# ZenHKD/ocr-vi-invoice

Measured on AMD Instinct MI355X. Metric: invoice images/sec end-to-end (det+rec), higher is better.
Workload: dtype f16x2

## Files before the change

### include/ocrvi.h

```cpp
#ifndef OCRVI_H
#define OCRVI_H

#include <stddef.h>
#include <stdint.h>

#ifdef __cplusplus
extern "C" {
#endif

#define OCRVI_OK 0
#define OCRVI_EINVAL (-1)
#define OCRVI_EHIP (-2)
#define OCRVI_ENOMEM (-3)
#define OCRVI_EBLOB (-4)
#define OCRVI_ERANGE (-5)

typedef enum { OCRVI_F32 = 0, OCRVI_BF16 = 1, OCRVI_F16 = 2, OCRVI_F16X2 = 3 } ocrvi_dtype;

const char* ocrvi_last_error(void);
int ocrvi_abi_version(void);

typedef struct ocrvi_det ocrvi_det;

typedef struct {
    int32_t dtype;
    float k;
    int32_t max_batch;
    int32_t backbone;
    int32_t no_dcn;
    int32_t reserved[3];
} ocrvi_det_cfg;

int ocrvi_det_create(int device, const void* blob, size_t blob_bytes, const ocrvi_det_cfg* cfg, ocrvi_det** out);
void ocrvi_det_destroy(ocrvi_det* h);
int ocrvi_det_workspace_bytes(const ocrvi_det* h, int N, int H, int W, size_t* bytes);
int ocrvi_det_forward(ocrvi_det* h, const float* x, int N, int H, int W,
                      float* binary, float* thresh, float* thresh_binary, float* bin_logits, float* thresh_logits,
                      void* workspace, size_t workspace_bytes, void* stream);
int ocrvi_det_binary_workspace_bytes(const ocrvi_det* h, int N, int H, int W, size_t* bytes);
int ocrvi_det_forward_binary(ocrvi_det* h, const float* x, int N, int H, int W, float* binary,
                             void* workspace, size_t workspace_bytes, void* stream);
int ocrvi_det_status(const ocrvi_det* h);
int ocrvi_det_debug_features(ocrvi_det* h, int N, int H, int W, float* c2, float* c3, float* c4, float* c5,
                             float* fused, void* workspace, size_t workspace_bytes, void* stream);

typedef struct ocrvi_rec ocrvi_rec;

typedef struct {
    int32_t dtype;
    int32_t dims[3];
    int32_t num_blocks[3];
    int32_t num_local[3];
    int32_t num_classes;
    int32_t blank_id;
    int32_t reserved[4];
} ocrvi_rec_cfg;

int ocrvi_rec_create(int device, const void* blob, size_t blob_bytes, const ocrvi_rec_cfg* cfg, ocrvi_rec** out);
void ocrvi_rec_destroy(ocrvi_rec* h);
int ocrvi_rec_workspace_bytes(const ocrvi_rec* h, int B, int H, int W, size_t* bytes);
int ocrvi_rec_forward(ocrvi_rec* h, const float* x, int B, int H, int W,
                      float* log_probs, int32_t* argmax_ids, int32_t* ids, int32_t* lens,
                      void* workspace, size_t workspace_bytes, void* stream);
int ocrvi_rec_status(const ocrvi_rec* h);
int ocrvi_rec_debug_features(ocrvi_rec* h, int B, int H, int W, float* backbone_norm, float* frm,
                             void* workspace, size_t workspace_bytes, void* stream);

int ocrvi_range_reset(int device, void* stream);
int ocrvi_range_flag(int device, int* raised);

int ocrvi_ctc_greedy(int device, const float* log_probs, int T, int B, int C, int blank_id,
                     int32_t* argmax_ids, int32_t* ids, int32_t* lens, void* stream);

int ocrvi_normalize_u8(int device, const uint8_t* images, int N, int H, int W, float* out, void* stream);
int ocrvi_resize_u8(int device, const uint8_t* src, int src_h, int src_w, uint8_t* dst, int dst_h, int dst_w, void* stream);
int ocrvi_crop_resize_normalize(int device, const uint8_t* images, int n_img, int H, int W, const int32_t* boxes, int B,
                                int out_h, int out_w, float* out, void* stream);

#define OCRVI_PAGE_ENTRY 4
int ocrvi_resize_normalize_pages(int device, const int64_t* pages, int n, int H, int W, float* out, void* stream);
int ocrvi_crop_resize_normalize_pages(int device, const int64_t* pages, int n_pages, const int32_t* boxes, int B, int out_h, int out_w,
                                      float* out, void* stream);

int ocrvi_four_point_transform(const double* pts , double* m_fwd , double* m_inv , int32_t* out_w, int32_t* out_h);
int ocrvi_warp_perspective_u8(int device, const uint8_t* src, int src_h, int src_w, const double* m_inv_host ,
                              uint8_t* dst, int dst_h, int dst_w, void* stream);
int ocrvi_warp_perspective_pages(int device, const int64_t* src_pages, const int64_t* dst_pages, const double* m_inv , int n,
                                 void* stream);

int ocrvi_min_area_quads(const int32_t* points, const int32_t* offs, int n, double* quads , int32_t* flags );
int ocrvi_quad_crops(const double* quads, const int32_t* flags, int n, const int32_t* page_ids, const int32_t* page_hw ,
                     int32_t* crops , double* m_inv );
int ocrvi_crop_quad_resize_normalize_pages(int device, const int64_t* pages, int n_pages, const int32_t* crops, const double* m_inv, int B,
                                           int out_h, int out_w, float* out, void* stream);
int ocrvi_crop_quad_resize_normalize(int device, const uint8_t* images, int n_img, int H, int W, const int32_t* crops, const double* m_inv,
                                     int B, int out_h, int out_w, float* out, void* stream);

int ocrvi_enhance_init(int device);
int ocrvi_enhance_tables(void* out, size_t cap, size_t* bytes);
int ocrvi_enhance_workspace_bytes(int h, int w, size_t* bytes);
int ocrvi_enhance_u8(int device, const uint8_t* src, int h, int w, uint8_t* dst, void* workspace, size_t workspace_bytes, void* stream);
int ocrvi_rgb_to_lab_u8(int device, const uint8_t* src, int h, int w, uint8_t* dst, void* stream);
int ocrvi_lab_to_rgb_u8(int device, const uint8_t* src, int h, int w, uint8_t* dst, void* stream);
#define OCRVI_CLAHE_WORKSPACE_BYTES 16384
int ocrvi_clahe_lab_u8(int device, const uint8_t* src, int h, int w, uint8_t* dst, void* workspace, size_t workspace_bytes, void* stream);
int ocrvi_nlm_lab_u8(int device, const uint8_t* src, int h, int w, uint8_t* dst, void* stream);
int ocrvi_sharpen_u8(int device, const uint8_t* src, int h, int w, uint8_t* dst, void* stream);

typedef struct {
    int32_t width, height, components;
    int32_t h_samp[3], v_samp[3];
    int32_t restart_interval;
    int32_t orientation;
    int32_t out_height, out_width;
    int32_t reserved;
    int64_t blocks;
    uint64_t stream_bytes;
    uint64_t workspace_bytes;
    uint16_t quant[3][64];
    char reason[160];
} ocrvi_jpeg_info_t;
int ocrvi_jpeg_info(const void* data, size_t n, ocrvi_jpeg_info_t* info);
int ocrvi_jpeg_parse(const void* data, size_t n, void* out, size_t cap, size_t* used);
#define OCRVI_JPEG_ENTRY 64
int ocrvi_jpeg_table_entry(const ocrvi_jpeg_info_t* info, size_t used, int64_t stream_offset, int64_t dst_offset, int64_t dst_stride,
                           int64_t workspace_offset, int64_t* entry);
int ocrvi_jpeg_decode_pages(int device, const void* records_dev, const int64_t* table_dev, int n_pages, void* dst_base, void* workspace,
                            size_t workspace_bytes, void* stream);

int ocrvi_jpeg_quant_tables(int quality, uint16_t* luma, uint16_t* chroma);
#define OCRVI_JPEG_HEADER_MAX 640
int ocrvi_jpeg_encode_header(int width, int height, int components, int subsampling, int quality, void* out, size_t cap, size_t* used);
int ocrvi_jpeg_encode_sizes(int width, int height, int components, int subsampling, int64_t* blocks, uint64_t* workspace_bytes,
                            uint64_t* scan_capacity, uint64_t* offsets);
#define OCRVI_JPEG_ENC_ENTRY 64
int ocrvi_jpeg_encode_table_entry(int width, int height, int components, int subsampling, int quality, int64_t src_offset, int64_t src_stride,
                                  int64_t out_offset, int64_t out_capacity, int64_t workspace_offset, int64_t* entry);
int ocrvi_jpeg_encode_pages(int device, const void* src_base, const int64_t* table_dev, int n_pages, void* out_base, int64_t* lengths_dev,
                            void* workspace, size_t workspace_bytes, void* stream);

#define OCRVI_OVERLAY_SEG 8
#define OCRVI_OVERLAY_PRIM 8
#define OCRVI_OVERLAY_MAX_COORD 16384
int ocrvi_overlay_segments(const int32_t* points, const int32_t* offs, const int32_t* page_boxes, const int32_t* page_pairs,
                           const int32_t* page_hw , int n_pages, uint32_t box_rgb, uint32_t label_rgb, int thickness,
                           int32_t* segs , int64_t seg_cap, int32_t* prims ,
                           int64_t prim_cap, int32_t* prim_offs , int64_t* n_segs, int64_t* n_prims);
int ocrvi_overlay_pages(int device, const int64_t* pages, int n_pages, const int32_t* prims, const int32_t* segs, const int32_t* prim_offs,
                        int max_h, int max_w, void* stream);

int ocrvi_db_postprocess(const float* prob, int H, int W, float thresh, float box_thresh, int max_candidates, float unclip_ratio,
                         float min_area, int32_t* points, int cap_points, int32_t* box_offsets, float* scores, int cap_boxes, int* n_boxes);

int ocrvi_unclip_polygon(const int32_t* pts, int n_pts, double distance, int32_t* out, int cap_pts, int* n_out);

int ocrvi_db_boxes_batch(const float* prob, int n_pages, int H, int W, float thresh, float box_thresh, int max_candidates,
                         float unclip_ratio, float min_area, double scale_w, double scale_h, int orig_h, int orig_w, int page_base,
                         int32_t* rects, float* scores, int cap_per_page, int32_t* counts, int threads);

int ocrvi_db_boxes_pages(const float* prob, int n_pages, int H, int W, float thresh, float box_thresh, int max_candidates, float unclip_ratio,
                         float min_area, const double* scale_w, const double* scale_h, const int32_t* orig_h, const int32_t* orig_w,
                         const int32_t* page_ids, int32_t* points, int cap_points, int32_t* box_offsets, int32_t* rects, float* scores,
                         int cap_per_page, int32_t* counts, int32_t* overflow, int threads);

size_t ocrvi_db_components_workspace_bytes(int n_pages, int H, int W);
int ocrvi_db_components(int device, const float* prob, int n_pages, int H, int W, float thresh, uint32_t* mask_bits, int32_t* comps,
                        int32_t* counts, int cap, long long* offsets, float* packed, long long pack_cap, void* workspace, void* stream);
int ocrvi_db_boxes_batch_sparse(const uint32_t* mask_bits, const int32_t* comps, const int32_t* comp_counts, int cap, const long long* offsets,
                                const float* packed, long long pack_cap, int n_pages, int H, int W, float box_thresh, int max_candidates,
                                float unclip_ratio, float min_area, double scale_w, double scale_h, int orig_h, int orig_w, int page_base,
                                int32_t* rects, float* scores, int cap_per_page, int32_t* counts, int threads, int32_t* skipped);

#define OCRVI_DB_TARGET_GT 0
#define OCRVI_DB_TARGET_MASK 1
#define OCRVI_DB_TARGET_THRESH 2
#define OCRVI_DB_TARGET_JOB 8
#define OCRVI_DB_TARGET_MAX_SIDE 16384
int ocrvi_db_target_jobs(const int32_t* sizes, const float* xy, const int32_t* poly_offsets, const int32_t* image_offsets, int n_images,
                         double shrink_ratio, int want_thresh, int32_t* jobs, int cap_jobs, int32_t* points, int cap_points, int32_t* n_jobs,
                         int32_t* n_points, int32_t* overflow, int threads);
int ocrvi_db_target_maps(int device, const int32_t* jobs, int n_jobs, const int32_t* points, int n_points, const int32_t* rows, int n, int S,
                         float thresh_max, float* gt, float* mask, float* thresh_map, float* thresh_mask, void* stream);
int ocrvi_resize_normalize_pad_pages(int device, const int64_t* pages, const int32_t* rows, int n, int S, float* out, void* stream);

#define OCRVI_DET_EVAL_RECORD_BYTES 104
#define OCRVI_DET_EVAL_TP 0
#define OCRVI_DET_EVAL_FP 1
#define OCRVI_DET_EVAL_FN 2
#define OCRVI_DET_EVAL_POSITIVES 3
#define OCRVI_DET_EVAL_NEGATIVES 4
#define OCRVI_DET_EVAL_K 5
#define OCRVI_DET_EVAL_POS_BCE 6
#define OCRVI_DET_EVAL_TOPK_BCE 7
#define OCRVI_DET_EVAL_DICE_INTER 8
#define OCRVI_DET_EVAL_PRED_MASK 9
#define OCRVI_DET_EVAL_GT_MASK 10
#define OCRVI_DET_EVAL_L1_NUM 11
#define OCRVI_DET_EVAL_THRESH_MASK 12
int ocrvi_det_eval_workspace_bytes(int N, int H, int W, size_t* bytes);
int ocrvi_det_eval(int device, const float* binary, const float* thresh, const float* thresh_binary, const float* bin_logits,
                   const float* gt, const float* mask, const float* thresh_map, const float* thresh_mask, int N, int H, int W,
                   double negative_ratio, void* record, void* workspace, size_t workspace_bytes, void* stream);

#define OCRVI_CTC_LOSS_MAX_TARGET 1024
int ocrvi_ctc_loss(int device, const float* log_probs, int T, int B, int C, const int32_t* targets, int Lmax, const int32_t* target_lengths,
                   const int32_t* input_lengths, int blank, double* nll, void* stream);

#define OCRVI_EDIT_DISTANCE_MAX_LEN 2048
int ocrvi_edit_distance(int device, const int32_t* pred_ids, int T, const int32_t* pred_lens, const int32_t* gt_ids, int G,
                        const int32_t* gt_lens, int B, int32_t* dist, void* stream);

int ocrvi_test_offset_conv(int device, int dtype, const float* x, const float* weight_host, const float* bias_host, int N, int C, int H, int W,
                           int stride, float* out, int iters, float* avg_ms);
int ocrvi_test_deform_conv(int device, int dtype, const float* x, const float* offset, const float* mask,
                           const float* weight_host, const float* bias_host, int N, int C, int H, int W, int Co,
                           int stride, int relu, float* out, int iters, float* avg_ms);
int ocrvi_test_deform_conv_res(int device, int dtype, const float* x, const float* offset, const float* mask,
                               const float* weight_host, const float* bias_host, const float* res, int N, int C, int H, int W, int Co,
                               int stride, int relu, float* out, int iters, float* avg_ms);
int ocrvi_test_deform_conv_raw(int device, int dtype, const float* x, const float* offset, const float* mask,
                               const float* weight_host, const float* bias_host, const float* res, int N, int C, int H, int W, int Co,
                               int stride, int relu, void* out_raw, float* out);
int ocrvi_test_dcn_plan(int dtype, int N, int C, int H, int W, int Co, int stride, int n_cu, int32_t plan[8]);
int ocrvi_test_conv(int device, int dtype, const float* x, const float* weight_host, const float* bias_host,
                    int N, int C, int H, int W, int Co, int ksize, int sh, int sw, int groups, int act, float* out,
                    int iters, float* avg_ms);
int ocrvi_test_conv_res(int device, int dtype, const float* x, const float* weight_host, const float* bias_host, const float* res, int N,
                        int C, int H, int W, int Co, int ksize, int res_mode, int act, float* out, int iters, float* avg_ms);
int ocrvi_test_bneck_tail(int device, const float* t1, const float* identity, const float* w2_host, const float* b2_host,
                          const float* w3_host, const float* b3_host, const float* w1_host, const float* b1_host, int N, int H, int W,
                          int no_phase_c, float* y_out, float* t1n_out, int iters, float* avg_ms);
int ocrvi_test_db_tail(int device, int dtype, const float* x, const float* dc1_w_bin_host, const float* dc1_b_bin_host,
                       const float* dc1_w_thr_host, const float* dc1_b_thr_host, const float* dc2_w_bin_host, const float* dc2_b_bin_host,
                       const float* dc2_w_thr_host, const float* dc2_b_thr_host, int N, int OH, int OW, int groups, int binary_only,
                       float* out, float* out2, int iters, float* avg_ms);
int ocrvi_test_gemm(int device, int dtype, const float* a, const float* weight_host, const float* bias_host, const float* res, int M,
                    int K, int N, int act, int res_post, int out_f32, float* out, int iters, float* avg_ms);
int ocrvi_test_gemm_raw(int device, int dtype, const float* a, const float* weight_host, const float* bias_host, const float* res, int M,
                        int K, int N, int act, int res_post, int out_f32, void* out_raw, float* out);
int ocrvi_test_ring_plan(int dtype, int amode, int M, int K, int N, int out_f32, int has_res, int n_cu, int32_t plan[8]);
int ocrvi_test_stem_pool(int device, int dtype, const float* x, const float* weight_host, const float* bias_host, int N, int H, int W, int fused,
                         float* out, int iters, float* avg_ms);
int ocrvi_test_attention(int device, int dtype, const float* qkv, int B, int N, int heads, float* out, int iters,
                         float* avg_ms);

int ocrvi_test_mlp(int device, int dtype, float* x, const float* ln_g_host, const float* ln_b_host, const float* w1_host, const float* b1_host,
                   const float* w2_host, const float* b2_host, const float* next_g_host, const float* next_b_host, int want_xn, int M, int D,
                   float* xn_out, int iters, float* avg_ms);
int ocrvi_test_mlp_raw(int device, int dtype, float* x, const float* ln_g_host, const float* ln_b_host, const float* w1_host, const float* b1_host,
                       const float* w2_host, const float* b2_host, const float* next_g_host, const float* next_b_host, int M, int D, void* xn_raw,
                       float* xn_out, int iters, float* avg_ms);
int ocrvi_test_pack_f16x2(const float* src, size_t n, void* dst, float* wscale);

int ocrvi_test_layernorm(int device, int dtype, const float* x, int x_f32, int out_f32, const float* gamma_host, const float* beta_host,
                         int rows, int D, float* out);
int ocrvi_test_frm_vertical(int device, int dtype, const float* kv, const float* vq_host, int B, int H, int W, int D, float* out);
int ocrvi_test_asf(int device, int dtype, const float* p2, const float* p3, const float* p4, const float* p5, const float* w_host,
                   const float* b_host, int N, int H, int W, float* out);
int ocrvi_test_maxpool(int device, int dtype, const float* x, int N, int C, int H, int W, float* out);
int ocrvi_test_db_maps(int device, const float* bin_logits, const float* thresh_logits, float k, float* binary, float* thresh,
                       float* thresh_binary, size_t n);
int ocrvi_test_ctc_logsoftmax(int device, const float* logits, int ld, int B, int T, int C, float* log_probs, int32_t* argmax_ids);

int ocrvi_prof_enable(int on);
int ocrvi_prof_reset(void);
int ocrvi_prof_report(char* buf, size_t cap);

#ifdef __cplusplus
}
#endif
#endif
```

### ocr_vi_invoice_amd/_lib.py

```python
from __future__ import annotations

import ctypes as C
import os
from typing import Optional

_HERE = os.path.dirname(os.path.abspath(__file__))
LIB_PATH = os.environ.get("OCRVI_LIB") or os.path.join(_HERE, "lib", "libocrvi.so")

OCRVI_F32, OCRVI_BF16, OCRVI_F16, OCRVI_F16X2 = 0, 1, 2, 3
DTYPES = {"f32": OCRVI_F32, "fp32": OCRVI_F32, "float32": OCRVI_F32, "bf16": OCRVI_BF16, "bfloat16": OCRVI_BF16,
          "f16": OCRVI_F16, "fp16": OCRVI_F16, "float16": OCRVI_F16,
          "f16x2": OCRVI_F16X2}
ABI_VERSION = 5

EXPORTS = [
    "ocrvi_last_error", "ocrvi_abi_version",
    "ocrvi_det_create", "ocrvi_det_destroy", "ocrvi_det_workspace_bytes", "ocrvi_det_forward", "ocrvi_det_debug_features",
    "ocrvi_rec_create", "ocrvi_rec_destroy", "ocrvi_rec_workspace_bytes", "ocrvi_rec_forward", "ocrvi_rec_debug_features",
    "ocrvi_ctc_greedy", "ocrvi_normalize_u8", "ocrvi_resize_u8", "ocrvi_crop_resize_normalize", "ocrvi_db_postprocess", "ocrvi_db_boxes_batch",
    "ocrvi_unclip_polygon", "ocrvi_db_components_workspace_bytes", "ocrvi_db_components", "ocrvi_db_boxes_batch_sparse",
    "ocrvi_test_deform_conv", "ocrvi_test_offset_conv", "ocrvi_test_conv", "ocrvi_test_gemm", "ocrvi_test_attention", "ocrvi_test_mlp", "ocrvi_test_stem_pool", "ocrvi_test_pack_f16x2",
    "ocrvi_prof_enable", "ocrvi_prof_reset", "ocrvi_prof_report",
    "ocrvi_det_status", "ocrvi_rec_status", "ocrvi_range_reset", "ocrvi_range_flag",
    "ocrvi_resize_normalize_pages", "ocrvi_crop_resize_normalize_pages", "ocrvi_db_boxes_pages",
    "ocrvi_det_binary_workspace_bytes", "ocrvi_det_forward_binary",
    "ocrvi_four_point_transform", "ocrvi_warp_perspective_u8", "ocrvi_warp_perspective_pages",
    "ocrvi_test_layernorm", "ocrvi_test_frm_vertical", "ocrvi_test_asf", "ocrvi_test_maxpool", "ocrvi_test_db_maps", "ocrvi_test_ctc_logsoftmax",
    "ocrvi_det_eval_workspace_bytes", "ocrvi_det_eval", "ocrvi_ctc_loss", "ocrvi_edit_distance",
    "ocrvi_test_deform_conv_res",
    "ocrvi_enhance_init", "ocrvi_enhance_tables", "ocrvi_enhance_workspace_bytes", "ocrvi_enhance_u8",
    "ocrvi_rgb_to_lab_u8", "ocrvi_lab_to_rgb_u8", "ocrvi_clahe_lab_u8", "ocrvi_nlm_lab_u8", "ocrvi_sharpen_u8",
    "ocrvi_min_area_quads", "ocrvi_quad_crops", "ocrvi_crop_quad_resize_normalize_pages", "ocrvi_crop_quad_resize_normalize",
    "ocrvi_jpeg_info", "ocrvi_jpeg_parse", "ocrvi_jpeg_table_entry", "ocrvi_jpeg_decode_pages",
    "ocrvi_test_conv_res", "ocrvi_test_db_tail",
    "ocrvi_db_target_jobs", "ocrvi_db_target_maps", "ocrvi_resize_normalize_pad_pages",
    "ocrvi_test_mlp_raw",
    "ocrvi_test_bneck_tail",
    "ocrvi_jpeg_quant_tables", "ocrvi_jpeg_encode_header", "ocrvi_jpeg_encode_sizes", "ocrvi_jpeg_encode_table_entry", "ocrvi_jpeg_encode_pages",
    "ocrvi_test_gemm_raw", "ocrvi_test_ring_plan",
    "ocrvi_overlay_segments", "ocrvi_overlay_pages",
    "ocrvi_test_deform_conv_raw", "ocrvi_test_dcn_plan",
]
PAGE_ENTRY = 4
DET_EVAL_RECORD_BYTES = 104
DET_EVAL_INT_SLOTS = ("tp", "fp", "fn", "positive_count", "negatives", "negative_count")
DET_EVAL_F64_SLOTS = ("pos_bce", "topk_bce", "dice_inter", "pred_mask", "gt_mask", "l1_num", "thresh_mask")
CTC_LOSS_MAX_TARGET = 1024
EDIT_DISTANCE_MAX_LEN = 2048
CLAHE_WORKSPACE_BYTES = 16384
ENHANCE_MIN_SIDE = 16
DB_TARGET_GT, DB_TARGET_MASK, DB_TARGET_THRESH = 0, 1, 2
DB_TARGET_JOB = 8
DB_TARGET_MAX_SIDE = 16384
JPEG_ENTRY = 64
JPEG_ENC_ENTRY = 64
JPEG_HEADER_MAX = 640
OVERLAY_SEG = 8
OVERLAY_PRIM = 8
OVERLAY_MAX_COORD = 16384


class DetCfg(C.Structure):
    _fields_ = [("dtype", C.c_int32), ("k", C.c_float), ("max_batch", C.c_int32), ("backbone", C.c_int32), ("no_dcn", C.c_int32),
                ("reserved", C.c_int32 * 3)]


class RecCfg(C.Structure):
    _fields_ = [("dtype", C.c_int32), ("dims", C.c_int32 * 3), ("num_blocks", C.c_int32 * 3), ("num_local", C.c_int32 * 3),
                ("num_classes", C.c_int32), ("blank_id", C.c_int32), ("reserved", C.c_int32 * 4)]


class JpegInfo(C.Structure):
    _fields_ = [("width", C.c_int32), ("height", C.c_int32), ("components", C.c_int32), ("h_samp", C.c_int32 * 3), ("v_samp", C.c_int32 * 3),
                ("restart_interval", C.c_int32), ("orientation", C.c_int32), ("out_height", C.c_int32), ("out_width", C.c_int32),
                ("reserved", C.c_int32), ("blocks", C.c_int64), ("stream_bytes", C.c_uint64), ("workspace_bytes", C.c_uint64),
                ("quant", (C.c_uint16 * 64) * 3), ("reason", C.c_char * 160)]


_lib: Optional[C.CDLL] = None


def load() -> C.CDLL:
    global _lib
    if _lib is not None:
        return _lib
    if not os.path.exists(LIB_PATH):
        raise RuntimeError(
            f"libocrvi.so not found at {LIB_PATH}: build it with `python -c 'import __graft_entry__ as g; g.build()'` "
            "(or `make -C ocr_vi_invoice_amd/csrc`).  There is no CPU fallback for the product path.")
    import torch
    lib = C.CDLL(LIB_PATH)
    vp, i32, f32p, i32p, sz = C.c_void_p, C.c_int, C.c_void_p, C.c_void_p, C.c_size_t
    lib.ocrvi_last_error.restype = C.c_char_p
    lib.ocrvi_last_error.argtypes = []
    lib.ocrvi_abi_version.restype = i32
    lib.ocrvi_det_create.argtypes = [i32, vp, sz, C.POINTER(DetCfg), C.POINTER(vp)]
    lib.ocrvi_det_destroy.argtypes = [vp]
    lib.ocrvi_det_destroy.restype = None
    lib.ocrvi_det_workspace_bytes.argtypes = [vp, i32, i32, i32, C.POINTER(sz)]
    lib.ocrvi_det_forward.argtypes = [vp, f32p, i32, i32, i32, f32p, f32p, f32p, f32p, f32p, vp, sz, vp]
    lib.ocrvi_det_binary_workspace_bytes.argtypes = [vp, i32, i32, i32, C.POINTER(sz)]
    lib.ocrvi_det_forward_binary.argtypes = [vp, f32p, i32, i32, i32, f32p, vp, sz, vp]
    lib.ocrvi_det_debug_features.argtypes = [vp, i32, i32, i32, f32p, f32p, f32p, f32p, f32p, vp, sz, vp]
    lib.ocrvi_rec_create.argtypes = [i32, vp, sz, C.POINTER(RecCfg), C.POINTER(vp)]
    lib.ocrvi_rec_destroy.argtypes = [vp]
    lib.ocrvi_rec_destroy.restype = None
    lib.ocrvi_rec_workspace_bytes.argtypes = [vp, i32, i32, i32, C.POINTER(sz)]
    lib.ocrvi_rec_forward.argtypes = [vp, f32p, i32, i32, i32, f32p, i32p, i32p, i32p, vp, sz, vp]
    lib.ocrvi_rec_debug_features.argtypes = [vp, i32, i32, i32, f32p, f32p, vp, sz, vp]
    lib.ocrvi_ctc_greedy.argtypes = [i32, f32p, i32, i32, i32, i32, i32p, i32p, i32p, vp]
    lib.ocrvi_normalize_u8.argtypes = [i32, vp, i32, i32, i32, f32p, vp]
    lib.ocrvi_resize_u8.argtypes = [i32, vp, i32, i32, vp, i32, i32, vp]
    lib.ocrvi_crop_resize_normalize.argtypes = [i32, vp, i32, i32, i32, i32p, i32, i32, i32, f32p, vp]
    lib.ocrvi_db_postprocess.argtypes = [vp, i32, i32, C.c_float, C.c_float, i32, C.c_float, C.c_float, vp, i32, vp, vp, i32, C.POINTER(i32)]
    lib.ocrvi_db_components_workspace_bytes.argtypes = [i32, i32, i32]
    lib.ocrvi_db_components_workspace_bytes.restype = sz
    lib.ocrvi_db_components.argtypes = [i32, vp, i32, i32, i32, C.c_float, vp, vp, vp, i32, vp, vp, C.c_longlong, vp, vp]
    lib.ocrvi_db_boxes_batch_sparse.argtypes = [vp, vp, vp, i32, vp, vp, C.c_longlong, i32, i32, i32, C.c_float, i32, C.c_float, C.c_float,
                                                C.c_double, C.c_double, i32, i32, i32, vp, vp, i32, vp, i32, vp]
    lib.ocrvi_unclip_polygon.argtypes = [vp, i32, C.c_double, vp, i32, C.POINTER(i32)]
    lib.ocrvi_db_boxes_batch.argtypes = [vp, i32, i32, i32, C.c_float, C.c_float, i32, C.c_float, C.c_float, C.c_double, C.c_double, i32, i32, i32,
                                         vp, vp, i32, vp, i32]
    lib.ocrvi_resize_normalize_pages.argtypes = [i32, vp, i32, i32, i32, f32p, vp]
    lib.ocrvi_crop_resize_normalize_pages.argtypes = [i32, vp, i32, i32p, i32, i32, i32, f32p, vp]
    lib.ocrvi_four_point_transform.argtypes = [vp, vp, vp, i32p, i32p]
    lib.ocrvi_warp_perspective_u8.argtypes = [i32, vp, i32, i32, vp, vp, i32, i32, vp]
    lib.ocrvi_warp_perspective_pages.argtypes = [i32, vp, vp, vp, i32, vp]
    lib.ocrvi_db_boxes_pages.argtypes = [vp, i32, i32, i32, C.c_float, C.c_float, i32, C.c_float, C.c_float, vp, vp, vp, vp, vp,
                                         vp, i32, vp, vp, vp, i32, vp, vp, i32]
    lib.ocrvi_test_deform_conv.argtypes = [i32, i32, f32p, f32p, f32p, vp, vp, i32, i32, i32, i32, i32, i32, i32, f32p, i32,
                                           C.POINTER(C.c_float)]
    lib.ocrvi_test_deform_conv_res.argtypes = [i32, i32, f32p, f32p, f32p, vp, vp, f32p, i32, i32, i32, i32, i32, i32, i32, f32p, i32,
                                               C.POINTER(C.c_float)]
    lib.ocrvi_test_offset_conv.argtypes = [i32, i32, f32p, vp, vp, i32, i32, i32, i32, i32, f32p, i32, C.POINTER(C.c_float)]
    lib.ocrvi_test_conv.argtypes = [i32, i32, f32p, vp, vp, i32, i32, i32, i32, i32, i32, i32, i32, i32, i32, f32p, i32,
                                    C.POINTER(C.c_float)]
    lib.ocrvi_test_conv_res.argtypes = [i32, i32, f32p, vp, vp, f32p, i32, i32, i32, i32, i32, i32, i32, i32, f32p, i32, C.POINTER(C.c_float)]
    lib.ocrvi_test_bneck_tail.argtypes = [i32, f32p, f32p, vp, vp, vp, vp, vp, vp, i32, i32, i32, i32, f32p, f32p, i32, C.POINTER(C.c_float)]
    lib.ocrvi_test_db_tail.argtypes = [i32, i32, f32p, vp, vp, vp, vp, vp, vp, vp, vp, i32, i32, i32, i32, i32, f32p, f32p, i32,
                                       C.POINTER(C.c_float)]
    lib.ocrvi_test_gemm.argtypes = [i32, i32, f32p, vp, vp, f32p, i32, i32, i32, i32, i32, i32, f32p, i32, C.POINTER(C.c_float)]
    lib.ocrvi_test_gemm_raw.argtypes = [i32, i32, f32p, vp, vp, f32p, i32, i32, i32, i32, i32, i32, vp, f32p]
    lib.ocrvi_test_ring_plan.argtypes = [i32, i32, i32, i32, i32, i32, i32, i32, C.POINTER(C.c_int32)]
    lib.ocrvi_test_deform_conv_raw.argtypes = [i32, i32, f32p, f32p, f32p, vp, vp, f32p, i32, i32, i32, i32, i32, i32, i32, vp, f32p]
    lib.ocrvi_test_dcn_plan.argtypes = [i32, i32, i32, i32, i32, i32, i32, i32, C.POINTER(C.c_int32)]
    lib.ocrvi_test_stem_pool.argtypes = [i32, i32, f32p, vp, vp, i32, i32, i32, i32, f32p, i32, C.POINTER(C.c_float)]
    lib.ocrvi_test_attention.argtypes = [i32, i32, f32p, i32, i32, i32, f32p, i32, C.POINTER(C.c_float)]
    lib.ocrvi_test_mlp.argtypes = [i32, i32, f32p, vp, vp, vp, vp, vp, vp, vp, vp, i32, i32, i32, f32p, i32, C.POINTER(C.c_float)]
    lib.ocrvi_test_mlp_raw.argtypes = [i32, i32, f32p, vp, vp, vp, vp, vp, vp, vp, vp, i32, i32, vp, f32p, i32, C.POINTER(C.c_float)]
    lib.ocrvi_test_pack_f16x2.argtypes = [f32p, sz, vp, C.POINTER(C.c_float)]
    lib.ocrvi_test_layernorm.argtypes = [i32, i32, f32p, i32, i32, vp, vp, i32, i32, f32p]
    lib.ocrvi_test_frm_vertical.argtypes = [i32, i32, f32p, vp, i32, i32, i32, i32, f32p]
    lib.ocrvi_test_asf.argtypes = [i32, i32, f32p, f32p, f32p, f32p, vp, vp, i32, i32, i32, f32p]
    lib.ocrvi_test_maxpool.argtypes = [i32, i32, f32p, i32, i32, i32, i32, f32p]
    lib.ocrvi_test_db_maps.argtypes = [i32, f32p, f32p, C.c_float, f32p, f32p, f32p, sz]
    lib.ocrvi_test_ctc_logsoftmax.argtypes = [i32, f32p, i32, i32, i32, i32, f32p, i32p]
    lib.ocrvi_det_eval_workspace_bytes.argtypes = [i32, i32, i32, C.POINTER(sz)]
    lib.ocrvi_det_eval.argtypes = [i32, f32p, f32p, f32p, f32p, f32p, f32p, f32p, f32p, i32, i32, i32, C.c_double, vp, vp, sz, vp]
    lib.ocrvi_ctc_loss.argtypes = [i32, f32p, i32, i32, i32, i32p, i32, i32p, i32p, i32, vp, vp]
    lib.ocrvi_edit_distance.argtypes = [i32, i32p, i32, i32p, i32p, i32, i32p, i32, i32p, vp]
    lib.ocrvi_enhance_init.argtypes = [i32]
    lib.ocrvi_enhance_tables.argtypes = [vp, sz, C.POINTER(sz)]
    lib.ocrvi_enhance_workspace_bytes.argtypes = [i32, i32, C.POINTER(sz)]
    lib.ocrvi_enhance_u8.argtypes = [i32, vp, i32, i32, vp, vp, sz, vp]
    for name in ("ocrvi_rgb_to_lab_u8", "ocrvi_lab_to_rgb_u8", "ocrvi_nlm_lab_u8", "ocrvi_sharpen_u8"):
        getattr(lib, name).argtypes = [i32, vp, i32, i32, vp, vp]
    lib.ocrvi_clahe_lab_u8.argtypes = [i32, vp, i32, i32, vp, vp, sz, vp]
    lib.ocrvi_min_area_quads.argtypes = [vp, vp, i32, vp, vp]
    lib.ocrvi_quad_crops.argtypes = [vp, vp, i32, vp, vp, vp, vp]
    lib.ocrvi_crop_quad_resize_normalize_pages.argtypes = [i32, vp, i32, i32p, vp, i32, i32, i32, f32p, vp]
    lib.ocrvi_crop_quad_resize_normalize.argtypes = [i32, vp, i32, i32, i32, i32p, vp, i32, i32, i32, f32p, vp]
    lib.ocrvi_jpeg_info.argtypes = [vp, sz, C.POINTER(JpegInfo)]
    lib.ocrvi_jpeg_parse.argtypes = [vp, sz, vp, sz, C.POINTER(sz)]
    lib.ocrvi_jpeg_table_entry.argtypes = [C.POINTER(JpegInfo), sz, C.c_int64, C.c_int64, C.c_int64, C.c_int64, vp]
    lib.ocrvi_jpeg_decode_pages.argtypes = [i32, vp, vp, i32, vp, vp, sz, vp]
    lib.ocrvi_jpeg_quant_tables.argtypes = [i32, vp, vp]
    lib.ocrvi_jpeg_encode_header.argtypes = [i32, i32, i32, i32, i32, vp, sz, C.POINTER(sz)]
    lib.ocrvi_jpeg_encode_sizes.argtypes = [i32, i32, i32, i32, C.POINTER(C.c_int64), C.POINTER(C.c_uint64), C.POINTER(C.c_uint64), vp]
    lib.ocrvi_jpeg_encode_table_entry.argtypes = [i32, i32, i32, i32, i32, C.c_int64, C.c_int64, C.c_int64, C.c_int64, C.c_int64, vp]
    lib.ocrvi_jpeg_encode_pages.argtypes = [i32, vp, vp, i32, vp, vp, vp, sz, vp]
    lib.ocrvi_overlay_segments.argtypes = [vp, vp, vp, vp, vp, i32, C.c_uint32, C.c_uint32, i32, vp, C.c_int64, vp, C.c_int64, vp,
                                           C.POINTER(C.c_int64), C.POINTER(C.c_int64)]
    lib.ocrvi_overlay_pages.argtypes = [i32, vp, i32, vp, vp, vp, i32, i32, vp]
    lib.ocrvi_db_target_jobs.argtypes = [vp, vp, vp, vp, i32, C.c_double, i32, vp, i32, vp, i32, C.POINTER(C.c_int32), C.POINTER(C.c_int32),
                                         C.POINTER(C.c_int32), i32]
    lib.ocrvi_db_target_maps.argtypes = [i32, vp, i32, vp, i32, vp, i32, i32, C.c_float, f32p, f32p, f32p, f32p, vp]
    lib.ocrvi_resize_normalize_pad_pages.argtypes = [i32, vp, vp, i32, i32, f32p, vp]
    lib.ocrvi_det_status.argtypes = [vp]
    lib.ocrvi_rec_status.argtypes = [vp]
    lib.ocrvi_range_reset.argtypes = [i32, vp]
    lib.ocrvi_range_flag.argtypes = [i32, C.POINTER(i32)]
    lib.ocrvi_prof_enable.argtypes = [i32]
    lib.ocrvi_prof_reset.argtypes = []
    lib.ocrvi_prof_report.argtypes = [C.c_char_p, sz]
    for name in EXPORTS:
        fn = getattr(lib, name)
        if name not in ("ocrvi_last_error", "ocrvi_det_destroy", "ocrvi_rec_destroy"):
            fn.restype = i32
    if lib.ocrvi_abi_version() != ABI_VERSION:
        raise RuntimeError(f"libocrvi ABI {lib.ocrvi_abi_version()} != binding {ABI_VERSION}: rebuild")
    _lib = lib
    return lib


def last_error() -> str:
    return load().ocrvi_last_error().decode("utf-8", "replace")


def check(rc: int) -> None:
    if rc == 0:
        return
    msg = last_error()
    if rc == -1:
        raise ValueError(msg)
    if rc == -3:
        raise MemoryError(msg)
    if rc == -5:
        raise OverflowError(msg)
    raise RuntimeError(f"libocrvi error {rc}: {msg}")


def dtype_code(dtype) -> int:
    if isinstance(dtype, int):
        return dtype
    try:
        return DTYPES[str(dtype).replace("torch.", "")]
    except KeyError:
        raise ValueError(f"unsupported compute dtype {dtype!r}; choose from f32, f16x2, bf16, f16") from None


def ptr(t) -> Optional[int]:
    return None if t is None else t.data_ptr()


def prof_report() -> dict:
    import json
    buf = C.create_string_buffer(1 << 20)
    check(load().ocrvi_prof_report(buf, len(buf)))
    return json.loads(buf.value.decode())
```

### ocr_vi_invoice_amd/csrc/kernels.h

```cpp
#pragma once
#include "common.h"

namespace ocrvi {

int k_nchw3_to_nhwc4_pad(int dtype, const float* x, void* y, int N, int H, int W, int pad_t, int pad_l, int Hp, int Wp, hipStream_t s);
int k_maxpool3x3s2(int dtype, const void* x, void* y, int N, int H, int W, int C, hipStream_t s);
bool stem_pool_eligible(int dtype, int cout, int Kp, int KH, int H, int W);
int k_stem_pool(int dtype, const void* xpad, const void* w, const float* bias, float wscale, void* y, int N, int H, int W, int Hp, int Wp,
                hipStream_t s);
int k_layernorm(int dtype, const void* x, int x_f32, void* out, int out_f32, const float* gamma, const float* beta, int rows, int D,
                hipStream_t s);
bool mlp_fused_eligible(int dtype, int D);
bool mlp_x2_eligible(int dtype, int D);
void pack_mlp_x2_stream(const float* w1, const float* w2, int D, std::vector<char>& out);
int k_mlp_x2(float* x, void* xn, const float* ln_g, const float* ln_b, const float* next_g, const float* next_b, const void* wstream, const float* b1,
             const float* b2, int M, int D, hipStream_t s);
void pack_mlp_stream(const float* w1, const float* w2, int D, int dtype, std::vector<char>& out);
int k_mlp_fused(int dtype, float* x, void* xn, const float* ln_g, const float* ln_b, const float* next_g, const float* next_b, const void* wstream,
                const float* b1, const float* b2, int M, int D, hipStream_t s);
int k_cast_from_f32(int dtype, const float* x, void* y, size_t n, hipStream_t s);
int k_nhwc_to_nchw_f32(int dtype, const void* x, float* y, int N, int H, int W, int C, int ld, int coff, hipStream_t s);

int k_attention(int dtype, const void* qkv, void* out, int B, int N, int heads, hipStream_t s, void* scratch = nullptr);
size_t attention_scratch_bytes(int dtype, int B, int N, int heads);
int k_frm_vertical(int dtype, const void* kv, const float* vq, void* out, int B, int H, int W, int D, hipStream_t s);

int k_asf(int dtype, const void* p2, const void* p3, const void* p4, const void* p5, const float* w, const float* b, float* scratch, void* out,
          int N, int H, int W, hipStream_t s);
size_t asf_scratch_bytes(int N, int H, int W);
int k_db_maps(const float* bin_logits, const float* thresh_logits, float k, float* binary, float* thresh, float* thresh_binary, size_t n,
              hipStream_t s);

int k_ctc_logsoftmax_argmax(const float* logits, int ld, float* log_probs, int32_t* argmax_ids, int B, int T, int C, hipStream_t s);
int k_ctc_argmax_tbc(const float* log_probs, int32_t* argmax_ids, int B, int T, int C, hipStream_t s);
int k_ctc_collapse(const int32_t* argmax_ids, int32_t* ids, int32_t* lens, int B, int T, int blank, hipStream_t s);

}
```

### ocr_vi_invoice_amd/csrc/mlp_x2.hip

```cpp
#include <stdlib.h>
#include <string.h>

#include "gemm_ring.h"
#include "kernels.h"

namespace ocrvi {
OCRVI_RANGE_FLAG_TU()

struct MlpX2Params {
    float* x = nullptr;
    void* xn = nullptr;
    const float* ln_g = nullptr;
    const float* ln_b = nullptr;
    const float* next_g = nullptr;
    const float* next_b = nullptr;
    const char* wstream = nullptr;
    const float* b1 = nullptr;
    const float* b2 = nullptr;
    int M = 0;
};

template <int D, int R, int TB, bool SPLIT>
__global__ __launch_bounds__(512 / TB, TB == 2 ? 1 : 2) void mlp_x2_kernel(const MlpX2Params p) {
    typedef f16x2_t T;
    typedef Mma<T>::u4v U;
    constexpr int NWV = 8 / TB, NT = 64 * NWV;
    constexpr int KS = D / 32;
    constexpr int NCH = 4 * D / 32;
    constexpr int NB2 = D / 16;
    constexpr int W1B = 32 * D * 4;
    constexpr int UNIT = SPLIT ? W1B : 2 * W1B;
    constexpr int IPW = UNIT / 1024 / NWV;
    constexpr int PF = R - 1;
    constexpr int NU = (NCH + 1) * (SPLIT ? 2 : 1);
    static_assert(UNIT % (1024 * NWV) == 0 && R >= 2, "ring geometry");
    extern __shared__ __attribute__((aligned(16))) char smem[];
    const unsigned lds0 = (unsigned)(size_t)(__attribute__((address_space(3))) char*)smem;
    float* const c_b1 = (float*)(smem + R * UNIT);
    float* const c_b2 = c_b1 + 4 * D;
    float* const c_g = c_b2 + D;
    float* const c_be = c_g + D;
    float* const c_ng = c_be + D;
    float* const c_nb = c_ng + D;

    const int tid = threadIdx.x, lane = tid & 63;
    const int wave = __builtin_amdgcn_readfirstlane(tid >> 6);
    const int lr = lane & 15, g = lane >> 4;
    const bool next_ln = p.next_g != nullptr;
    for (int i = tid; i < 4 * D; i += NT) c_b1[i] = p.b1[i];
    for (int i = tid; i < D; i += NT) {
        c_b2[i] = p.b2[i];
        c_g[i] = p.ln_g[i];
        c_be[i] = p.ln_b[i];
        c_ng[i] = next_ln ? p.next_g[i] : 1.f;
        c_nb[i] = next_ln ? p.next_b[i] : 0.f;
    }
    const float* const tail = (const float*)(p.wstream + (size_t)(NCH + 1) * 2 * W1B);
    const float ws1 = tail[0], ws2 = tail[1];
    __syncthreads();

    const int ntiles = (p.M + 127) >> 7;
    const int G = gridDim.x;
    const int my_tiles = (ntiles - (int)blockIdx.x + G - 1) / G;

    const char* const wbase = uniform_ptr(p.wstream);
    int prod_slot = 0, prod_mod = 0, cons_slot = 0;
    auto issue_unit = [&]() {
        const char* src = wbase + (size_t)prod_mod * UNIT + wave * 1024;
        const unsigned dst = lds0 + prod_slot * UNIT + wave * 1024;
#pragma unroll
        for (int j = 0; j < IPW; ++j) glds16(src + j * (NWV * 1024), (unsigned)lane * 16u, __builtin_amdgcn_readfirstlane(dst + j * (NWV * 1024)));
        prod_slot = prod_slot + 1 == R ? 0 : prod_slot + 1;
        prod_mod = prod_mod + 1 == NU ? 0 : prod_mod + 1;
    };
    auto next_unit = [&]() -> const char* {
        wait_vm_barrier<(PF - 1) * IPW>();
        issue_unit();
        const char* s = smem + cons_slot * UNIT;
        cons_slot = cons_slot + 1 == R ? 0 : cons_slot + 1;
        return s;
    };
    for (int i = 0; i < PF; ++i) issue_unit();
    const int sw = swz128(lr);
    const int fo0 = ((2 * g) ^ sw) << 4, fo1 = ((2 * g + 1) ^ sw) << 4;
    unsigned long long range_mask = 0;

    for (int t = 0; t < my_tiles; ++t) {
        const int tile = (int)blockIdx.x + t * G;
        const int tok0 = tile * 128 + wave * (16 * TB);
        U xH[KS][TB], xL[KS][TB];
#pragma unroll
        for (int b = 0; b < TB; ++b) {
            float xv[KS][8];
            const int tok = min(tok0 + 16 * b + lr, p.M - 1);
            const float* xr = p.x + (size_t)tok * D + 8 * g;
#pragma unroll
            for (int ks = 0; ks < KS; ++ks) {
                const float4 v0 = *(const float4*)(xr + 32 * ks), v1 = *(const float4*)(xr + 32 * ks + 4);
                xv[ks][0] = v0.x; xv[ks][1] = v0.y; xv[ks][2] = v0.z; xv[ks][3] = v0.w;
                xv[ks][4] = v1.x; xv[ks][5] = v1.y; xv[ks][6] = v1.z; xv[ks][7] = v1.w;
            }
            float sum = 0.f;
#pragma unroll
            for (int ks = 0; ks < KS; ++ks)
#pragma unroll
                for (int e = 0; e < 8; ++e) sum += xv[ks][e];
            sum += __shfl_xor(sum, 16);
            sum += __shfl_xor(sum, 32);
            const float mean = sum / (float)D;
            float sq = 0.f;
#pragma unroll
            for (int ks = 0; ks < KS; ++ks)
#pragma unroll
                for (int e = 0; e < 8; ++e) { const float d = xv[ks][e] - mean; sq += d * d; }
            sq += __shfl_xor(sq, 16);
            sq += __shfl_xor(sq, 32);
            const float rstd = rsqrtf(sq / (float)D + 1e-5f);
#pragma unroll
            for (int ks = 0; ks < KS; ++ks) {
                float o[8];
#pragma unroll
                for (int q = 0; q < 2; ++q) {
                    const float4 gv = *(const float4*)(c_g + 32 * ks + 8 * g + 4 * q), bv = *(const float4*)(c_be + 32 * ks + 8 * g + 4 * q);
                    o[4 * q] = (xv[ks][4 * q] - mean) * rstd * gv.x + bv.x;
                    o[4 * q + 1] = (xv[ks][4 * q + 1] - mean) * rstd * gv.y + bv.y;
                    o[4 * q + 2] = (xv[ks][4 * q + 2] - mean) * rstd * gv.z + bv.z;
                    o[4 * q + 3] = (xv[ks][4 * q + 3] - mean) * rstd * gv.w + bv.w;
                }
                const uint4 c0 = Chunk<T>::pack(o), c1 = Chunk<T>::pack(o + 4);
                Mma<T>::regroup(c0, c1, xH[ks][b], xL[ks][b]);
            }
        }
        wait_vm_only<0>();

        f32x4 acc2[NB2][TB];
#pragma unroll
        for (int a = 0; a < NB2; ++a)
#pragma unroll
            for (int b = 0; b < TB; ++b) acc2[a][b] = (f32x4){0.f, 0.f, 0.f, 0.f};

        f32x4 hacc[2][TB], hprev[2][TB];
        constexpr int NV = 8 * TB;
        auto gelu_vals = [&](int i0, int i1, const float* bp) {
#pragma unroll
            for (int i = i0; i < i1; ++i) {
                const int b = i >> 3, a = (i >> 2) & 1, r = i & 3;
                hprev[a][b][r] = gelu_erf(hprev[a][b][r] * ws1 + bp[16 * a + r]);
            }
        };
        auto g1 = [&](const char* U1, bool with_gelu, const float* bv) {
#pragma unroll
            for (int a = 0; a < 2; ++a)
#pragma unroll
                for (int b = 0; b < TB; ++b) hacc[a][b] = (f32x4){0.f, 0.f, 0.f, 0.f};
            constexpr int P1 = TB == 2 ? 1 : 2;
            uint4 wr[P1 + 1][2][2];
            auto rd1 = [&](int ks, int set) {
#pragma unroll
                for (int a = 0; a < 2; ++a) {
                    const char* r = U1 + (ks * 32 + 16 * a + lr) * 128;
                    wr[set][a][0] = *(const uint4*)(r + fo0);
                    wr[set][a][1] = *(const uint4*)(r + fo1);
                }
            };
#pragma unroll
            for (int i = 0; i < P1; ++i) rd1(i, i);
            __builtin_amdgcn_sched_barrier(0);
#pragma unroll
            for (int ks = 0; ks < KS; ++ks) {
                if (ks + P1 < KS) rd1(ks + P1, (ks + P1) % (P1 + 1));
                __builtin_amdgcn_sched_barrier(0);
#pragma unroll
                for (int a = 0; a < 2; ++a)
#pragma unroll
                    for (int b = 0; b < TB; ++b)
                        Mma<T>::three(Mma<T>::as_u4v(wr[ks % (P1 + 1)][a][0]), Mma<T>::as_u4v(wr[ks % (P1 + 1)][a][1]), xH[ks][b], xL[ks][b], hacc[a][b]);
                if (with_gelu) gelu_vals(NV * ks / KS, NV * (ks + 1) / KS, bv);
                __builtin_amdgcn_sched_barrier(0);
            }
        };
        auto g2 = [&](const char* U2) {
            constexpr int GB = 2 / TB, NG = NB2 / GB, PFG = 2;
            uint4 w2r[PFG + 1][GB][2];
            auto rd2 = [&](int grp, int set) {
#pragma unroll
                for (int i = 0; i < GB; ++i) {
                    const char* r = U2 + (16 * (grp * GB + i) + lr) * 128;
                    w2r[set][i][0] = *(const uint4*)(r + fo0);
                    w2r[set][i][1] = *(const uint4*)(r + fo1);
                }
            };
#pragma unroll
            for (int i = 0; i < PFG; ++i) rd2(i, i);
            U hH[TB], hL[TB];
#pragma unroll
            for (int b = 0; b < TB; ++b) {
                const float h0[4] = {hprev[0][b][0], hprev[0][b][1], hprev[0][b][2], hprev[0][b][3]};
                const float h1[4] = {hprev[1][b][0], hprev[1][b][1], hprev[1][b][2], hprev[1][b][3]};
                range_mask |= f16x2_out_of_range(h0) | f16x2_out_of_range(h1);
                const uint4 c0 = Chunk<T>::pack(h0), c1 = Chunk<T>::pack(h1);
                Mma<T>::regroup(c0, c1, hH[b], hL[b]);
            }
            __builtin_amdgcn_sched_barrier(0);
#pragma unroll
            for (int grp = 0; grp < NG; ++grp) {
                if (grp + PFG < NG) rd2(grp + PFG, (grp + PFG) % (PFG + 1));
                __builtin_amdgcn_sched_barrier(0);
#pragma unroll
                for (int i = 0; i < GB; ++i)
#pragma unroll
                    for (int b = 0; b < TB; ++b)
                        Mma<T>::three(Mma<T>::as_u4v(w2r[grp % (PFG + 1)][i][0]), Mma<T>::as_u4v(w2r[grp % (PFG + 1)][i][1]), hH[b], hL[b], acc2[grp * GB + i][b]);
                __builtin_amdgcn_sched_barrier(0);
            }
        };
        auto keep = [&]() {
#pragma unroll
            for (int a = 0; a < 2; ++a)
#pragma unroll
                for (int b = 0; b < TB; ++b) hprev[a][b] = hacc[a][b];
        };
        auto second = [&](const char* U1) -> const char* {
            if constexpr (SPLIT) {
                return next_unit();
            } else {
                return U1 + W1B;
            }
        };
        auto bias_of = [&](int c) {
            int l = threadIdx.x;
            asm volatile("" : "+v"(l));
            return c_b1 + 32 * c + 4 * ((l & 63) >> 4);
        };
        {
            const char* const U1 = next_unit();
            g1(U1, false, bias_of(0));
            (void)second(U1);
        }
        keep();
        for (int k = 1; k < NCH; ++k) {
            const char* const U1 = next_unit();
            g1(U1, true, bias_of(k - 1));
            g2(second(U1));
            keep();
        }
        {
            const char* const U1 = next_unit();
            gelu_vals(0, NV, bias_of(NCH - 1));
            g2(second(U1));
        }

        const int pn_tok = lane >> 2, pn_g = lane & 3;
        const int pn_src = 4 * (16 * pn_g + pn_tok);
#pragma unroll
        for (int b = 0; b < TB; ++b) {
#pragma unroll
            for (int a = 0; a < NB2; ++a)
#pragma unroll
                for (int r = 0; r < 4; ++r)
                    acc2[a][b][r] = __int_as_float(__builtin_amdgcn_ds_bpermute(pn_src, __float_as_int(acc2[a][b][r])));
            const int tok = tok0 + 16 * b + pn_tok;
            const bool ok = tok < p.M;
            float* xr = p.x + (size_t)(ok ? tok : 0) * D + 4 * pn_g;
            float sum = 0.f;
            float4 rvs[NB2];
#pragma unroll
            for (int a = 0; a < NB2; ++a) rvs[a] = *(const float4*)(xr + 16 * a);
#pragma unroll
            for (int a = 0; a < NB2; ++a) {
                const float4 bv2 = *(const float4*)(c_b2 + 16 * a + 4 * pn_g);
                const float4 rv = rvs[a];
                f32x4 v = acc2[a][b];
                v[0] = v[0] * ws2 + bv2.x + rv.x; v[1] = v[1] * ws2 + bv2.y + rv.y; v[2] = v[2] * ws2 + bv2.z + rv.z; v[3] = v[3] * ws2 + bv2.w + rv.w;
                acc2[a][b] = v;
                if (ok) *(float4*)(xr + 16 * a) = make_float4(v[0], v[1], v[2], v[3]);
                sum += v[0] + v[1] + v[2] + v[3];
            }
            if (p.xn) {
                float mean = 0.f, rstd = 1.f;
                if (next_ln) {
                    sum += __shfl_xor(sum, 1);
                    sum += __shfl_xor(sum, 2);
                    mean = sum / (float)D;
                    float sq = 0.f;
#pragma unroll
                    for (int a = 0; a < NB2; ++a)
#pragma unroll
                        for (int r = 0; r < 4; ++r) { const float d = acc2[a][b][r] - mean; sq += d * d; }
                    sq += __shfl_xor(sq, 1);
                    sq += __shfl_xor(sq, 2);
                    rstd = rsqrtf(sq / (float)D + 1e-5f);
                }
                T* nr = (T*)p.xn + (size_t)(ok ? tok : 0) * D + 4 * pn_g;
#pragma unroll
                for (int a = 0; a < NB2; ++a) {
                    const float4 gv = *(const float4*)(c_ng + 16 * a + 4 * pn_g), bvn = *(const float4*)(c_nb + 16 * a + 4 * pn_g);
                    const f32x4 v = acc2[a][b];
                    const float o[4] = {(v[0] - mean) * rstd * gv.x + bvn.x, (v[1] - mean) * rstd * gv.y + bvn.y, (v[2] - mean) * rstd * gv.z + bvn.z,
                                        (v[3] - mean) * rstd * gv.w + bvn.w};
                    range_mask |= f16x2_out_of_range(o);
                    if (ok) *(uint4*)(nr + 16 * a) = Chunk<T>::pack(o);
                }
            }
        }
    }
    wait_vm_only<0>();
    f16x2_raise(range_mask);
}

bool mlp_x2_eligible(int dtype, int D) {
    static const bool off = getenv("OCRVI_MLP_X2") && atoi(getenv("OCRVI_MLP_X2")) == 0;
    return !off && dtype == OCRVI_F16X2 && (D == 128 || D == 256 || D == 384);
}

static float x2_scale(const float* w, size_t n) {
    float mx = 0.f;
    for (size_t i = 0; i < n; ++i) mx = std::max(mx, fabsf(w[i]));
    if (!(mx > 0.f) || !std::isfinite(mx)) return 1.f;
    int e = 0;
    (void)frexpf(mx, &e);
    return ldexpf(1.0f, std::min(std::max(14 - e, -100), 100));
}

void pack_mlp_x2_stream(const float* w1, const float* w2, int D, std::vector<char>& out) {
    const int H4 = 4 * D, NCH = H4 / 32, KS = D / 32;
    const float s1 = x2_scale(w1, (size_t)H4 * D), s2 = x2_scale(w2, (size_t)D * H4);
    const size_t rows_per_unit = (size_t)KS * 32 + D, nrows = (size_t)(NCH + 1) * rows_per_unit;
    std::vector<float> buf(nrows * 32, 0.f);
    std::vector<int> rowidx(nrows);
    size_t o = 0, ri = 0;
    for (int k = 0; k <= NCH; ++k) {
        for (int ks = 0; ks < KS; ++ks)
            for (int r = 0; r < 32; ++r) {
                rowidx[ri++] = ks * 32 + r;
                for (int e = 0; e < 32; ++e, ++o)
                    if (k < NCH) buf[o] = w1[(size_t)(32 * k + r) * D + 32 * ks + e] * s1;
            }
        for (int n = 0; n < D; ++n) {
            rowidx[ri++] = n;
            for (int pos = 0; pos < 32; ++pos, ++o) {
                const int g = pos >> 3, j = pos & 7;
                if (k >= 1) buf[o] = w2[(size_t)n * H4 + 32 * (k - 1) + 16 * (j >> 2) + 4 * g + (j & 3)] * s2;
            }
        }
    }
    std::vector<char> chunks(buf.size() * 4);
    convert_to_dtype(buf.data(), buf.size(), OCRVI_F16X2, chunks.data());
    out.assign(chunks.size() + 8, 0);
    for (size_t r = 0; r < nrows; ++r) {
        const uint64_t* src = (const uint64_t*)(chunks.data() + r * 128);
        uint64_t q[16];
        for (int k = 0; k < 4; ++k) {
            q[4 * k] = src[4 * k]; q[4 * k + 1] = src[4 * k + 2]; q[4 * k + 2] = src[4 * k + 1]; q[4 * k + 3] = src[4 * k + 3];
        }
        const int row = rowidx[r], sw = ((row >> 1) & 1) | (((row >> 3) & 1) << 2);
        uint64_t* dst = (uint64_t*)(out.data() + r * 128);
        for (int ch = 0; ch < 8; ++ch) {
            dst[2 * (ch ^ sw)] = q[2 * ch];
            dst[2 * (ch ^ sw) + 1] = q[2 * ch + 1];
        }
    }
    const float tail[2] = {1.0f / s1, 1.0f / s2};
    memcpy(out.data() + chunks.size(), tail, 8);
}

template <int D, int R, int TB, bool SPLIT>
static int launch_mlp_x2(const MlpX2Params& p, hipStream_t s) {
    const int smem = R * (SPLIT ? 128 : 256) * D + 9 * D * 4;
    auto kern = mlp_x2_kernel<D, R, TB, SPLIT>;
    OCRVI_TRY(ensure_max_smem((const void*)kern, smem));
    int n_cu = 0;
    OCRVI_TRY(device_cus(&n_cu));
    const int ntiles = (p.M + 127) / 128;
    int grid = std::min(ntiles, n_cu);
    grid = cdiv(ntiles, cdiv(ntiles, grid));
    hipLaunchKernelGGL(kern, dim3(grid), dim3(512 / TB), smem, s, p);
    OCRVI_HIP(hipGetLastError());
    return OCRVI_OK;
}

int k_mlp_x2(float* x, void* xn, const float* ln_g, const float* ln_b, const float* next_g, const float* next_b, const void* wstream, const float* b1,
             const float* b2, int M, int D, hipStream_t s) {
    OCRVI_CHECK((D == 128 || D == 256 || D == 384) && x && ln_g && ln_b && wstream && b1 && b2 && M > 0 && M < (1 << 24), OCRVI_EINVAL,
                "mlp_x2: bad argument (D %d, M %d)", D, M);
    MlpX2Params p;
    p.x = x; p.xn = xn; p.ln_g = ln_g; p.ln_b = ln_b; p.next_g = next_g; p.next_b = next_b; p.wstream = (const char*)wstream; p.b1 = b1; p.b2 = b2; p.M = M;
    char tag[64];
    snprintf(tag, sizeof(tag), "mlp_fused_d%d_f16x2", D);
    ProfScope ps(tag, 2.0 * M * 8.0 * D * D, (double)M * D * (8.0 + (xn ? 4.0 : 0.0)) + 8.0 * D * D * 4.0, s);
    if (D == 128) return launch_mlp_x2<128, 4, 1, false>(p, s);
    if (D == 256) return launch_mlp_x2<256, 2, 1, false>(p, s);
    return launch_mlp_x2<384, 3, 2, true>(p, s);
}

}
```

### ocr_vi_invoice_amd/csrc/rec_model.hip

```cpp
#include <stdlib.h>
#include <string.h>

#include <algorithm>
#include <memory>

#include "model.h"

using namespace ocrvi;

namespace {
struct LNw { float *g = nullptr, *b = nullptr; };
struct MlpW {
    ConvLayer fc1, fc2;
    void* stream = nullptr;
    float *b1 = nullptr, *b2 = nullptr;
};
struct BlockW {
    bool local = false;
    LNw n1, n2;
    ConvLayer conv1, conv2;
    ConvLayer qkv, proj;
    MlpW mlp;
};
}

struct ocrvi_rec {
    int device = 0;
    ocrvi_rec_cfg cfg{};
    DeviceStore store;
    ConvLayer stem1, stem2;
    std::vector<BlockW> blocks[3];
    ConvLayer merge[2];
    LNw backbone_norm;
    LNw h_norm, h_norm2, v_norm_kv, v_norm2;
    ConvLayer h_qkv, h_proj, v_kv, v_proj, head;
    MlpW h_mlp, v_mlp;
    float* vq = nullptr;
    void *tap_bn = nullptr, *tap_frm = nullptr;
    RangeWatch range;
};

static int load_ln(DeviceStore& st, const Blob& b, const std::string& name, int d, LNw* ln) {
    OCRVI_TRY(load_vec(st, b, name + ".w", d, &ln->g));
    return load_vec(st, b, name + ".b", d, &ln->b);
}
static int load_lin(DeviceStore& st, const Blob& b, const std::string& name, int cout, int cin, int dt, ConvLayer* L, const float* extra = nullptr) {
    return load_conv(st, b, name, cout, cin, 0, 1, AM_CONV1, dt, true, L, extra);
}
static int load_mlp(DeviceStore& st, const Blob& b, const std::string& name, int d, int dt, MlpW* m) {
    OCRVI_TRY(load_lin(st, b, name + ".fc1", 4 * d, d, dt, &m->fc1));
    OCRVI_TRY(load_lin(st, b, name + ".fc2", d, 4 * d, dt, &m->fc2));
    static const bool fuse = !(getenv("OCRVI_MLP_FUSED") && atoi(getenv("OCRVI_MLP_FUSED")) == 0);
    if (fuse && mlp_fused_eligible(dt, d)) {
        const BlobTensor *w1 = nullptr, *b1 = nullptr, *w2 = nullptr, *b2 = nullptr;
        OCRVI_TRY(b.get(name + ".fc1.w", 4 * d, d, 0, 0, &w1));
        OCRVI_TRY(b.get(name + ".fc1.b", 4 * d, 0, 0, 0, &b1));
        OCRVI_TRY(b.get(name + ".fc2.w", d, 4 * d, 0, 0, &w2));
        OCRVI_TRY(b.get(name + ".fc2.b", d, 0, 0, 0, &b2));
        std::vector<char> packed;
        pack_mlp_stream(w1->data, w2->data, d, dt, packed);
        OCRVI_TRY(st.upload(packed.data(), packed.size(), &m->stream));
        OCRVI_TRY(st.upload(b1->data, (size_t)4 * d * 4, (void**)&m->b1));
        OCRVI_TRY(st.upload(b2->data, (size_t)d * 4, (void**)&m->b2));
    }
    return OCRVI_OK;
}

extern "C" int ocrvi_rec_create(int device, const void* blob_p, size_t blob_bytes, const ocrvi_rec_cfg* cfg, ocrvi_rec** out) {
    OCRVI_CHECK(cfg && out, OCRVI_EINVAL, "rec_create: null argument");
    OCRVI_CHECK(dtype_valid(cfg->dtype), OCRVI_EINVAL, "rec_create: bad dtype %d", cfg->dtype);
    for (int s = 0; s < 3; ++s)
        OCRVI_CHECK(cfg->dims[s] > 0 && cfg->dims[s] % 32 == 0 && cfg->num_blocks[s] > 0 && cfg->num_local[s] >= 0 &&
                        cfg->num_local[s] <= cfg->num_blocks[s],
                    OCRVI_EINVAL, "rec_create: bad stage %d config (dims must be multiples of 32)", s);
    OCRVI_CHECK(cfg->num_classes > 0 && cfg->num_classes % 4 == 0 && cfg->num_classes <= 1024, OCRVI_EINVAL,
                "rec_create: num_classes=%d must be a multiple of 4 and <= 1024", cfg->num_classes);
    DeviceGuard dg(device);
    OCRVI_HIP(dg.err);
    Blob blob;
    OCRVI_TRY(blob.parse(blob_p, blob_bytes));
    std::unique_ptr<ocrvi_rec> h(new ocrvi_rec);
    h->device = device;
    h->cfg = *cfg;
    const int dt = cfg->dtype;
    DeviceStore& st = h->store;
    const int d0 = cfg->dims[0], mid = d0 / 2;
    OCRVI_TRY(load_conv(st, blob, "stem.conv1", mid, 3, 3, 1, AM_ROWS, dt, true, &h->stem1));
    OCRVI_TRY(load_conv(st, blob, "stem.conv2", d0, mid, 3, 1, AM_CONV3, dt, true, &h->stem2));
    for (int s = 0; s < 3; ++s) {
        const int d = cfg->dims[s];
        h->blocks[s].resize(cfg->num_blocks[s]);
        for (int b = 0; b < cfg->num_blocks[s]; ++b) {
            BlockW& bw = h->blocks[s][b];
            const std::string p = "stages." + std::to_string(s) + ".blocks." + std::to_string(b);
            bw.local = b < cfg->num_local[s];
            OCRVI_TRY(load_ln(st, blob, p + ".norm1", d, &bw.n1));
            OCRVI_TRY(load_ln(st, blob, p + ".norm2", d, &bw.n2));
            if (bw.local) {
                const int groups = d / 32;
                OCRVI_TRY(load_conv(st, blob, p + ".mixer.conv1", d, 32, 3, groups, AM_CONV3, dt, true, &bw.conv1));
                OCRVI_TRY(load_conv(st, blob, p + ".mixer.conv2", d, 32, 3, groups, AM_CONV3, dt, true, &bw.conv2));
            } else {
                OCRVI_TRY(load_lin(st, blob, p + ".mixer.qkv", 3 * d, d, dt, &bw.qkv));
                OCRVI_TRY(load_lin(st, blob, p + ".mixer.proj", d, d, dt, &bw.proj));
            }
            OCRVI_TRY(load_mlp(st, blob, p + ".mlp", d, dt, &bw.mlp));
        }
        if (s < 2) OCRVI_TRY(load_conv(st, blob, "merges." + std::to_string(s), cfg->dims[s + 1], d, 3, 1, AM_CONV3, dt, true, &h->merge[s]));
    }
    const int d = cfg->dims[2];
    OCRVI_TRY(load_ln(st, blob, "backbone_norm", d, &h->backbone_norm));
    OCRVI_TRY(load_ln(st, blob, "frm.h_norm", d, &h->h_norm));
    OCRVI_TRY(load_ln(st, blob, "frm.h_norm2", d, &h->h_norm2));
    OCRVI_TRY(load_ln(st, blob, "frm.v_norm_kv", d, &h->v_norm_kv));
    OCRVI_TRY(load_ln(st, blob, "frm.v_norm2", d, &h->v_norm2));
    OCRVI_TRY(load_lin(st, blob, "frm.h_qkv", 3 * d, d, dt, &h->h_qkv));
    OCRVI_TRY(load_lin(st, blob, "frm.h_proj", d, d, dt, &h->h_proj));
    OCRVI_TRY(load_lin(st, blob, "frm.v_kv", 2 * d, d, dt, &h->v_kv));
    const BlobTensor* tok = nullptr;
    OCRVI_TRY(blob.get("frm.select_token", d, 0, 0, 0, &tok));
    OCRVI_TRY(load_lin(st, blob, "frm.v_proj", d, d, dt, &h->v_proj, tok->data));
    OCRVI_TRY(load_mlp(st, blob, "frm.h_mlp", d, dt, &h->h_mlp));
    OCRVI_TRY(load_mlp(st, blob, "frm.v_mlp", d, dt, &h->v_mlp));
    OCRVI_TRY(load_vec(st, blob, "frm.vq", d, &h->vq));
    OCRVI_TRY(load_lin(st, blob, "head", cfg->num_classes, d, dt, &h->head));
    OCRVI_TRY(finish_create(dt, h->range));
    *out = h.release();
    return OCRVI_OK;
}

extern "C" void ocrvi_rec_destroy(ocrvi_rec* h) {
    if (!h) return;
    DeviceGuard dg(h->device);
    delete h;
}

static int check_rec_shape(const ocrvi_rec* h, int B, int H, int W) {
    OCRVI_CHECK(h, OCRVI_EINVAL, "rec: null handle");
    OCRVI_CHECK(B > 0 && H > 0 && W > 0 && H % 16 == 0 && W % 4 == 0, OCRVI_EINVAL,
                "rec: input (B=%d,3,%d,%d) needs H %% 16 == 0 and W %% 4 == 0", B, H, W);
    const int tok = (H / 4) * (W / 4) / 2, tok_max = dtype_size(h->cfg.dtype) == 2 ? 1024 : 4096;
    OCRVI_CHECK(tok <= tok_max && H / 16 <= 8, OCRVI_EINVAL,
                "rec: %dx%d gives %d tokens in the first global-attention stage (at most %d in this mode) or more than 8 rows after the backbone", H, W, tok, tok_max);
    OCRVI_CHECK((size_t)B * (H / 2) * (W / 2) < ((size_t)1 << 23), OCRVI_EINVAL, "rec: batch of %d %dx%d crops too large for one call (chunk it)", B, H, W);
    return OCRVI_OK;
}

static int ln(Runner& r, const Tensor& x, const Tensor& y, const LNw& w) {
    if (r.dry()) return OCRVI_OK;
    return k_layernorm(r.dtype, x.p, x.f32, y.p, y.f32, w.g, w.b, (int)x.pixels(), x.c, r.stream);
}
static Tensor view(const Tensor& t, int n, int h, int w, int c) { return wrap(t.p, n, h, w, c, t.f32); }
static int attention(Runner& r, const Tensor& qkv, const Tensor& out, int seqs, int len, int heads) {
    const size_t mk = r.arena.mark(), sb = attention_scratch_bytes(r.dtype, seqs, len, heads);
    void* asc = sb ? r.arena.alloc(sb) : nullptr;
    if (!r.dry()) OCRVI_TRY(k_attention(r.dtype, qkv.p, out.p, seqs, len, heads, r.stream, asc));
    r.arena.release(mk);
    return OCRVI_OK;
}

static const LNw kCast{};
static int mlp_block(Runner& r, const Tensor& x, const Tensor& xn, const Tensor& hb, const LNw& n, const MlpW& m, int d, const LNw* next = nullptr,
                     bool* xn_done = nullptr) {
    const int rows = (int)x.pixels();
    if (xn_done) *xn_done = false;
    if (m.stream) {
        if (xn_done) *xn_done = next != nullptr;
        if (r.dry()) return OCRVI_OK;
        return k_mlp_fused(r.dtype, (float*)x.p, next ? xn.p : nullptr, n.g, n.b, next ? next->g : nullptr, next ? next->b : nullptr, m.stream, m.b1, m.b2,
                           rows, d, r.stream);
    }
    OCRVI_TRY(ln(r, x, xn, n));
    ConvOpts o1;
    o1.act = ACT_GELU;
    OCRVI_TRY(conv(r, m.fc1, view(xn, rows, 1, 1, d), view(hb, rows, 1, 1, 4 * d), o1));
    ConvOpts o2;
    o2.res = &x;
    o2.res_mode = RES_SAME;
    return conv(r, m.fc2, view(hb, rows, 1, 1, 4 * d), view(x, rows, 1, 1, d), o2);
}

static int rec_run(ocrvi_rec* h, Runner& r, const float* x, int B, int H, int W, float* log_probs, int32_t* argmax_ids, int32_t* ids,
                   int32_t* lens) {
    const ocrvi_rec_cfg& c = h->cfg;
    const int dt = c.dtype;
    const bool lowp = dt != OCRVI_F32;
    int Hs = H / 4, Ws = W / 4;
    const int T = Ws;
    size_t max_tok_d = 0, max_tok = 0;
    {
        int hh = Hs;
        for (int s = 0; s < 3; ++s) {
            const size_t tok = (size_t)B * hh * Ws;
            max_tok = std::max(max_tok, tok);
            max_tok_d = std::max(max_tok_d, tok * c.dims[s]);
            if (s < 2) hh /= 2;
        }
    }
    const int Hp = H + 2, Wp = W + 8;
    Tensor xpad = r.alloc(B, Hp, Wp, 4);
    Tensor s1 = r.alloc(B, H / 2, W / 2, c.dims[0] / 2);
    void* X[2] = {r.arena.alloc(max_tok_d * 4), r.arena.alloc(max_tok_d * 4)};
    void* XN = r.arena.alloc(max_tok_d * dtype_size(dt));
    void* T1 = r.arena.alloc(max_tok_d * dtype_size(dt));
    void* BIG = r.arena.alloc(max_tok_d * 4 * dtype_size(dt));
    const int d2 = c.dims[2];
    Tensor logits = r.alloc(B * T, 1, 1, c.num_classes, true);
    int32_t* am_buf = (int32_t*)r.arena.alloc((size_t)B * T * 4);

    if (!r.dry()) OCRVI_TRY(k_nchw3_to_nhwc4_pad(dt, x, xpad.p, B, H, W, 1, 1, Hp, Wp, r.stream));
    {
        ConvOpts o;
        o.sh = o.sw = 2; o.pad = 1; o.act = ACT_GELU; o.Hp = Hp; o.Wp = Wp;
        OCRVI_TRY(conv(r, h->stem1, xpad, s1, o));
    }
    int cur = 0;
    Tensor xs = wrap(X[cur], B, Hs, Ws, c.dims[0], true);
    {
        ConvOpts o;
        o.sh = o.sw = 2; o.pad = 1; o.act = ACT_GELU;
        OCRVI_TRY(conv(r, h->stem2, s1, xs, o));
    }
    for (int s = 0; s < 3; ++s) {
        const int d = c.dims[s];
        const int rows = B * Hs * Ws;
        const Tensor xn = wrap(XN, B, Hs, Ws, d, false), t1 = wrap(T1, B, Hs, Ws, d, false), big = wrap(BIG, rows, 1, 1, 4 * d, false);
        bool xn_ready = false;
        const int nblk = (int)h->blocks[s].size();
        for (int bi = 0; bi < nblk; ++bi) {
            const BlockW& bw = h->blocks[s][bi];
            if (!xn_ready) OCRVI_TRY(ln(r, xs, xn, bw.n1));
            if (bw.local) {
                ConvOpts o;
                o.pad = 1; o.act = ACT_GELU;
                OCRVI_TRY(conv(r, bw.conv1, xn, t1, o));
                o.res = &xs; o.res_mode = RES_SAME; o.res_post = 1;
                OCRVI_TRY(conv(r, bw.conv2, t1, xs, o));
            } else {
                ConvOpts o;
                OCRVI_TRY(conv(r, bw.qkv, view(xn, rows, 1, 1, d), view(big, rows, 1, 1, 3 * d), o));
                OCRVI_TRY(attention(r, big, t1, B, Hs * Ws, d / 32));
                o.res = &xs; o.res_mode = RES_SAME;
                OCRVI_TRY(conv(r, bw.proj, view(t1, rows, 1, 1, d), view(xs, rows, 1, 1, d), o));
            }
            const LNw* next = bi + 1 < nblk ? &h->blocks[s][bi + 1].n1 : ((s < 2 && lowp) ? &kCast : nullptr);
            OCRVI_TRY(mlp_block(r, view(xs, rows, 1, 1, d), xn, big, bw.n2, bw.mlp, d, next, &xn_ready));
        }
        if (s < 2) {
            Tensor src = xn;
            if (lowp) {
                if (!xn_ready && !r.dry()) OCRVI_TRY(k_cast_from_f32(dt, (const float*)xs.p, xn.p, (size_t)rows * d, r.stream));
            } else {
                src = xs; src.f32 = false;
            }
            Tensor nx = wrap(X[cur ^ 1], B, Hs / 2, Ws, c.dims[s + 1], true);
            ConvOpts o;
            o.sh = 2; o.sw = 1; o.pad = 1;
            OCRVI_TRY(conv(r, h->merge[s], src, nx, o));
            xs = nx;
            cur ^= 1;
            Hs /= 2;
        }
    }
    const int rows = B * Hs * Ws;
    const Tensor bn = wrap(X[cur ^ 1], rows, 1, 1, d2, true);
    OCRVI_TRY(ln(r, view(xs, rows, 1, 1, d2), bn, h->backbone_norm));
    h->tap_bn = bn.p;
    const Tensor xr = wrap(X[cur], rows, 1, 1, d2, true);
    const Tensor xn = wrap(XN, rows, 1, 1, d2, false), t1 = wrap(T1, rows, 1, 1, d2, false), big = wrap(BIG, rows, 1, 1, 4 * d2, false);
    OCRVI_TRY(ln(r, bn, xn, h->h_norm));
    {
        ConvOpts o;
        OCRVI_TRY(conv(r, h->h_qkv, xn, view(big, rows, 1, 1, 3 * d2), o));
        OCRVI_TRY(attention(r, big, t1, B * Hs, Ws, d2 / 32));
        o.res = &bn; o.res_mode = RES_SAME;
        OCRVI_TRY(conv(r, h->h_proj, t1, xr, o));
    }
    bool xn_ready = false;
    OCRVI_TRY(mlp_block(r, xr, xn, big, h->h_norm2, h->h_mlp, d2, &h->v_norm_kv, &xn_ready));
    if (!xn_ready) OCRVI_TRY(ln(r, xr, xn, h->v_norm_kv));
    const int cols = B * Ws;
    const Tensor tq = wrap(r.arena.alloc((size_t)cols * d2 * 4), cols, 1, 1, d2, true);
    {
        ConvOpts o;
        OCRVI_TRY(conv(r, h->v_kv, xn, view(big, rows, 1, 1, 2 * d2), o));
        if (!r.dry()) OCRVI_TRY(k_frm_vertical(dt, big.p, h->vq, t1.p, B, Hs, Ws, d2, r.stream));
        OCRVI_TRY(conv(r, h->v_proj, view(t1, cols, 1, 1, d2), tq, o));
    }
    OCRVI_TRY(mlp_block(r, tq, view(xn, cols, 1, 1, d2), big, h->v_norm2, h->v_mlp, d2, lowp ? &kCast : nullptr, &xn_ready));
    h->tap_frm = tq.p;
    Tensor hin = view(xn, cols, 1, 1, d2);
    if (lowp) {
        if (!xn_ready && !r.dry()) OCRVI_TRY(k_cast_from_f32(dt, (const float*)tq.p, xn.p, (size_t)cols * d2, r.stream));
    } else {
        hin = tq; hin.f32 = false;
    }
    {
        ConvOpts o;
        OCRVI_TRY(conv(r, h->head, hin, logits, o));
    }
    if (!r.dry()) {
        int32_t* am = argmax_ids ? argmax_ids : am_buf;
        OCRVI_TRY(k_ctc_logsoftmax_argmax((const float*)logits.p, c.num_classes, log_probs, am, B, T, c.num_classes, r.stream));
        if (ids || lens) OCRVI_TRY(k_ctc_collapse(am, ids, lens, B, T, c.blank_id, r.stream));
    }
    return OCRVI_OK;
}

extern "C" int ocrvi_rec_workspace_bytes(const ocrvi_rec* h, int B, int H, int W, size_t* bytes) {
    return plan_workspace("rec_workspace_bytes", h, bytes, [&] { return check_rec_shape(h, B, H, W); }, [&](Runner& r) {
        return rec_run(const_cast<ocrvi_rec*>(h), r, nullptr, B, H, W, nullptr, nullptr, nullptr, nullptr);
    });
}

extern "C" int ocrvi_rec_forward(ocrvi_rec* h, const float* x, int B, int H, int W, float* log_probs, int32_t* argmax_ids, int32_t* ids,
                                 int32_t* lens, void* workspace, size_t workspace_bytes, void* stream) {
    return run_forward("rec_forward", h, x && workspace, "null input/workspace", workspace, workspace_bytes, stream,
                       [&] { return check_rec_shape(h, B, H, W); },
                       [&](Runner& r) { return rec_run(h, r, x, B, H, W, log_probs, argmax_ids, ids, lens); });
}

extern "C" int ocrvi_rec_status(const ocrvi_rec* h) {
    OCRVI_CHECK(h, OCRVI_EINVAL, "rec_status: null handle");
    return h->range.status("rec");
}

extern "C" int ocrvi_rec_debug_features(ocrvi_rec* h, int B, int H, int W, float* backbone_norm, float* frm, void* workspace,
                                        size_t workspace_bytes, void* stream) {
    OCRVI_TRY(check_rec_shape(h, B, H, W));
    OCRVI_CHECK(h->tap_bn && h->tap_frm, OCRVI_EINVAL, "rec_debug_features: no forward has run");
    DeviceGuard dg(h->device);
    OCRVI_HIP(dg.err);
    (void)workspace; (void)workspace_bytes;
    const int d = h->cfg.dims[2];
    const size_t ntok = (size_t)B * (H / 16) * (W / 4), ncol = (size_t)B * (W / 4);
    if (backbone_norm) OCRVI_HIP(hipMemcpyAsync(backbone_norm, h->tap_bn, ntok * d * 4, hipMemcpyDeviceToDevice, (hipStream_t)stream));
    if (frm) OCRVI_HIP(hipMemcpyAsync(frm, h->tap_frm, ncol * d * 4, hipMemcpyDeviceToDevice, (hipStream_t)stream));
    return OCRVI_OK;
}

extern "C" int ocrvi_ctc_greedy(int device, const float* log_probs, int T, int B, int C, int blank_id, int32_t* argmax_ids, int32_t* ids,
                                int32_t* lens, void* stream) {
    OCRVI_CHECK(log_probs && argmax_ids, OCRVI_EINVAL, "ctc_greedy: log_probs and argmax_ids are required");
    DeviceGuard dg(device);
    OCRVI_HIP(dg.err);
    OCRVI_TRY(k_ctc_argmax_tbc(log_probs, argmax_ids, B, T, C, (hipStream_t)stream));
    if (ids || lens) OCRVI_TRY(k_ctc_collapse(argmax_ids, ids, lens, B, T, blank_id, (hipStream_t)stream));
    return OCRVI_OK;
}
```

Baseline: 327.6.

## Fuse attention output projection, residual and LayerNorm into f16x2 MLP kernel

```diff
diff --git a/include/ocrvi.h b/include/ocrvi.h
--- a/include/ocrvi.h
+++ b/include/ocrvi.h
@@ -250,6 +250,10 @@
 int ocrvi_test_mlp_raw(int device, int dtype, float* x, const float* ln_g_host, const float* ln_b_host, const float* w1_host, const float* b1_host,
                        const float* w2_host, const float* b2_host, const float* next_g_host, const float* next_b_host, int M, int D, void* xn_raw,
                        float* xn_out, int iters, float* avg_ms);
+int ocrvi_test_mlp_chain(int device, float* x, const float* a, const float* wp_host, const float* bp_host, const float* ln_g_host,
+                         const float* ln_b_host, const float* w1_host, const float* b1_host, const float* w2_host, const float* b2_host,
+                         const float* next_g_host, const float* next_b_host, int M, int D, int grid_cap, int fused, void* xn_raw, float* xn_out,
+                         int reps, float* avg_ms);
 int ocrvi_test_pack_f16x2(const float* src, size_t n, void* dst, float* wscale);
 
 int ocrvi_test_layernorm(int device, int dtype, const float* x, int x_f32, int out_f32, const float* gamma_host, const float* beta_host,
diff --git a/ocr_vi_invoice_amd/_lib.py b/ocr_vi_invoice_amd/_lib.py
--- a/ocr_vi_invoice_amd/_lib.py
+++ b/ocr_vi_invoice_amd/_lib.py
@@ -40,6 +40,7 @@
     "ocrvi_test_gemm_raw", "ocrvi_test_ring_plan",
     "ocrvi_overlay_segments", "ocrvi_overlay_pages",
     "ocrvi_test_deform_conv_raw", "ocrvi_test_dcn_plan",
+    "ocrvi_test_mlp_chain",
 ]
 PAGE_ENTRY = 4
 DET_EVAL_RECORD_BYTES = 104
@@ -148,6 +149,7 @@
     lib.ocrvi_test_attention.argtypes = [i32, i32, f32p, i32, i32, i32, f32p, i32, C.POINTER(C.c_float)]
     lib.ocrvi_test_mlp.argtypes = [i32, i32, f32p, vp, vp, vp, vp, vp, vp, vp, vp, i32, i32, i32, f32p, i32, C.POINTER(C.c_float)]
     lib.ocrvi_test_mlp_raw.argtypes = [i32, i32, f32p, vp, vp, vp, vp, vp, vp, vp, vp, i32, i32, vp, f32p, i32, C.POINTER(C.c_float)]
+    lib.ocrvi_test_mlp_chain.argtypes = [i32, f32p, f32p] + [vp] * 10 + [i32, i32, i32, i32, vp, f32p, i32, C.POINTER(C.c_float)]
     lib.ocrvi_test_pack_f16x2.argtypes = [f32p, sz, vp, C.POINTER(C.c_float)]
     lib.ocrvi_test_layernorm.argtypes = [i32, i32, f32p, i32, i32, vp, vp, i32, i32, f32p]
     lib.ocrvi_test_frm_vertical.argtypes = [i32, i32, f32p, vp, i32, i32, i32, i32, f32p]
diff --git a/ocr_vi_invoice_amd/csrc/kernels.h b/ocr_vi_invoice_amd/csrc/kernels.h
--- a/ocr_vi_invoice_amd/csrc/kernels.h
+++ b/ocr_vi_invoice_amd/csrc/kernels.h
@@ -11,10 +11,15 @@
 int k_layernorm(int dtype, const void* x, int x_f32, void* out, int out_f32, const float* gamma, const float* beta, int rows, int D,
                 hipStream_t s);
 bool mlp_fused_eligible(int dtype, int D);
+struct MlpProj {
+    const void* a = nullptr;
+    const float* bias = nullptr;
+    const float* res = nullptr;
+};
 bool mlp_x2_eligible(int dtype, int D);
-void pack_mlp_x2_stream(const float* w1, const float* w2, int D, std::vector<char>& out);
+void pack_mlp_x2_stream(const float* w1, const float* w2, int D, std::vector<char>& out, const float* wproj = nullptr);
 int k_mlp_x2(float* x, void* xn, const float* ln_g, const float* ln_b, const float* next_g, const float* next_b, const void* wstream, const float* b1,
-             const float* b2, int M, int D, hipStream_t s);
+             const float* b2, int M, int D, hipStream_t s, const MlpProj* proj = nullptr, int grid_cap = 0);
 void pack_mlp_stream(const float* w1, const float* w2, int D, int dtype, std::vector<char>& out);
 int k_mlp_fused(int dtype, float* x, void* xn, const float* ln_g, const float* ln_b, const float* next_g, const float* next_b, const void* wstream,
                 const float* b1, const float* b2, int M, int D, hipStream_t s);
diff --git a/ocr_vi_invoice_amd/csrc/mlp_x2.hip b/ocr_vi_invoice_amd/csrc/mlp_x2.hip
--- a/ocr_vi_invoice_amd/csrc/mlp_x2.hip
+++ b/ocr_vi_invoice_amd/csrc/mlp_x2.hip
@@ -18,9 +18,35 @@
     const float* b1 = nullptr;
     const float* b2 = nullptr;
     int M = 0;
+    const void* a = nullptr;
+    const float* bp = nullptr;
+    const float* xres = nullptr;
 };
 
-template <int D, int R, int TB, bool SPLIT>
+__device__ __forceinline__ int lane_here() {
+    int l;
+    asm volatile("v_mbcnt_lo_u32_b32 %0, -1, 0\n\tv_mbcnt_hi_u32_b32 %0, -1, %0" : "=v"(l));
+    return l;
+}
+
+__device__ __forceinline__ float lane_xor_sum(float v, int lane, int m1, int m2) {
+    v += __int_as_float(__builtin_amdgcn_ds_bpermute((lane ^ m1) << 2, __float_as_int(v)));
+    return v + __int_as_float(__builtin_amdgcn_ds_bpermute((lane ^ m2) << 2, __float_as_int(v)));
+}
+
+template <typename P>
+__device__ __forceinline__ P* lane_ptr(P* ubase, unsigned byte_off) {
+    const unsigned long long b = (unsigned long long)ubase;
+    const unsigned blo = __builtin_amdgcn_readfirstlane((unsigned)b), bhi = __builtin_amdgcn_readfirstlane((unsigned)(b >> 32));
+    unsigned lo, hi;
+    asm volatile("v_add_co_u32 %0, vcc, %2, %3\n\tv_mov_b32 %1, %4\n\tv_addc_co_u32 %1, vcc, 0, %1, vcc"
+                 : "=&v"(lo), "=&v"(hi)
+                 : "s"(blo), "v"(byte_off), "s"(bhi)
+                 : "vcc");
+    return (P*)(((unsigned long long)hi << 32) | lo);
+}
+
+template <int D, int R, int TB, bool SPLIT, bool PROJ>
 __global__ __launch_bounds__(512 / TB, TB == 2 ? 1 : 2) void mlp_x2_kernel(const MlpX2Params p) {
     typedef f16x2_t T;
     typedef Mma<T>::u4v U;
@@ -32,7 +58,8 @@
     constexpr int UNIT = SPLIT ? W1B : 2 * W1B;
     constexpr int IPW = UNIT / 1024 / NWV;
     constexpr int PF = R - 1;
-    constexpr int NU = (NCH + 1) * (SPLIT ? 2 : 1);
+    constexpr int NPU = PROJ ? (SPLIT ? KS : KS / 2) : 0;
+    constexpr int NU = NPU + (NCH + 1) * (SPLIT ? 2 : 1);
     static_assert(UNIT % (1024 * NWV) == 0 && R >= 2, "ring geometry");
     extern __shared__ __attribute__((aligned(16))) char smem[];
     const unsigned lds0 = (unsigned)(size_t)(__attribute__((address_space(3))) char*)smem;
@@ -42,6 +69,7 @@
     float* const c_be = c_g + D;
     float* const c_ng = c_be + D;
     float* const c_nb = c_ng + D;
+    float* const c_bp = c_nb + D;
 
     const int tid = threadIdx.x, lane = tid & 63;
     const int wave = __builtin_amdgcn_readfirstlane(tid >> 6);
@@ -54,9 +82,12 @@
         c_be[i] = p.ln_b[i];
         c_ng[i] = next_ln ? p.next_g[i] : 1.f;
         c_nb[i] = next_ln ? p.next_b[i] : 0.f;
+        if constexpr (PROJ) c_bp[i] = p.bp[i];
     }
-    const float* const tail = (const float*)(p.wstream + (size_t)(NCH + 1) * 2 * W1B);
+    const float* const tail = (const float*)(p.wstream + (size_t)NU * UNIT);
     const float ws1 = tail[0], ws2 = tail[1];
+    float wsp = 1.f;
+    if constexpr (PROJ) wsp = __uint_as_float(__builtin_amdgcn_readfirstlane(__float_as_uint(tail[2])));
     __syncthreads();
 
     const int ntiles = (p.M + 127) >> 7;
@@ -89,6 +120,16 @@
         const int tile = (int)blockIdx.x + t * G;
         const int tok0 = tile * 128 + wave * (16 * TB);
         U xH[KS][TB], xL[KS][TB];
+        if constexpr (PROJ) {
+#pragma unroll
+            for (int b = 0; b < TB; ++b) {
+                const int lq = lane_here();
+                const int tok = min(tok0 + 16 * b + (lq & 15), p.M - 1);
+                const char* ar = (const char*)p.a + ((size_t)tok * D + 8 * ((lq & 63) >> 4)) * 4;
+#pragma unroll
+                for (int ks = 0; ks < KS; ++ks) Mma<T>::regroup(*(const uint4*)(ar + 128 * ks), *(const uint4*)(ar + 128 * ks + 16), xH[ks][b], xL[ks][b]);
+            }
+        } else {
 #pragma unroll
         for (int b = 0; b < TB; ++b) {
             float xv[KS][8];
@@ -131,6 +172,7 @@
                 Mma<T>::regroup(c0, c1, xH[ks][b], xL[ks][b]);
             }
         }
+        }
         wait_vm_only<0>();
 
         f32x4 acc2[NB2][TB];
@@ -179,7 +221,7 @@
                 __builtin_amdgcn_sched_barrier(0);
             }
         };
-        auto g2 = [&](const char* U2) {
+        auto g2f = [&](const char* U2, const U (&hH)[TB], const U (&hL)[TB], auto&& make_frags) {
             constexpr int GB = 2 / TB, NG = NB2 / GB, PFG = 2;
             uint4 w2r[PFG + 1][GB][2];
             auto rd2 = [&](int grp, int set) {
@@ -192,15 +234,7 @@
             };
 #pragma unroll
             for (int i = 0; i < PFG; ++i) rd2(i, i);
-            U hH[TB], hL[TB];
-#pragma unroll
-            for (int b = 0; b < TB; ++b) {
-                const float h0[4] = {hprev[0][b][0], hprev[0][b][1], hprev[0][b][2], hprev[0][b][3]};
-                const float h1[4] = {hprev[1][b][0], hprev[1][b][1], hprev[1][b][2], hprev[1][b][3]};
-                range_mask |= f16x2_out_of_range(h0) | f16x2_out_of_range(h1);
-                const uint4 c0 = Chunk<T>::pack(h0), c1 = Chunk<T>::pack(h1);
-                Mma<T>::regroup(c0, c1, hH[b], hL[b]);
-            }
+            make_frags();
             __builtin_amdgcn_sched_barrier(0);
 #pragma unroll
             for (int grp = 0; grp < NG; ++grp) {
@@ -213,6 +247,19 @@
                         Mma<T>::three(Mma<T>::as_u4v(w2r[grp % (PFG + 1)][i][0]), Mma<T>::as_u4v(w2r[grp % (PFG + 1)][i][1]), hH[b], hL[b], acc2[grp * GB + i][b]);
                 __builtin_amdgcn_sched_barrier(0);
             }
+        };
+        auto g2 = [&](const char* U2) {
+            U hH[TB], hL[TB];
+            g2f(U2, hH, hL, [&]() {
+#pragma unroll
+                for (int b = 0; b < TB; ++b) {
+                    const float h0[4] = {hprev[0][b][0], hprev[0][b][1], hprev[0][b][2], hprev[0][b][3]};
+                    const float h1[4] = {hprev[1][b][0], hprev[1][b][1], hprev[1][b][2], hprev[1][b][3]};
+                    range_mask |= f16x2_out_of_range(h0) | f16x2_out_of_range(h1);
+                    const uint4 c0 = Chunk<T>::pack(h0), c1 = Chunk<T>::pack(h1);
+                    Mma<T>::regroup(c0, c1, hH[b], hL[b]);
+                }
+            });
         };
         auto keep = [&]() {
 #pragma unroll
@@ -229,9 +276,69 @@
         };
         auto bias_of = [&](int c) {
             int l = threadIdx.x;
-            asm volatile("" : "+v"(l));
+            if constexpr (PROJ) l = lane_here(); else asm volatile("" : "+v"(l));
             return c_b1 + 32 * c + 4 * ((l & 63) >> 4);
         };
+        if constexpr (PROJ) {
+            const char* Up = nullptr;
+#pragma unroll
+            for (int ks = 0; ks < KS; ++ks) {
+                if (SPLIT || (ks & 1) == 0) Up = next_unit(); else Up += W1B;
+                g2f(Up, xH[ks], xL[ks], []() {});
+            }
+#pragma unroll
+            for (int b = 0; b < TB; ++b) {
+                const int lq = lane_here();
+                const int gq = (lq & 63) >> 4;
+                const int tok = tok0 + 16 * b + (lq & 15);
+                const bool ok = tok < p.M;
+                const size_t ro = (size_t)(ok ? tok : 0) * D + 4 * gq;
+                constexpr int RB = TB == 2 ? 6 : NB2;
+                float4 rvs[RB];
+                float sum = 0.f;
+#pragma unroll
+                for (int a = 0; a < NB2; ++a) {
+                    if (a % RB == 0) {
+#pragma unroll
+                        for (int i = 0; i < RB; ++i) rvs[i] = *(const float4*)(p.xres + ro + 16 * (a + i));
+                    }
+                    const float4 bv = *(const float4*)(c_bp + 16 * a + 4 * gq);
+                    const float4 rv = rvs[a % RB];
+                    f32x4 v = acc2[a][b];
+                    v[0] = v[0] * wsp + bv.x + rv.x; v[1] = v[1] * wsp + bv.y + rv.y; v[2] = v[2] * wsp + bv.z + rv.z; v[3] = v[3] * wsp + bv.w + rv.w;
+                    acc2[a][b] = v;
+                    if (ok) *(float4*)(p.x + ro + 16 * a) = make_float4(v[0], v[1], v[2], v[3]);
+                    sum += v[0] + v[1] + v[2] + v[3];
+                }
+                sum = lane_xor_sum(sum, lq & 63, 16, 32);
+                const float mean = sum / (float)D;
+                float sq = 0.f;
+#pragma unroll
+                for (int a = 0; a < NB2; ++a)
+#pragma unroll
+                    for (int r = 0; r < 4; ++r) { const float d = acc2[a][b][r] - mean; sq += d * d; }
+                sq = lane_xor_sum(sq, lq & 63, 16, 32);
+                const float rstd = rsqrtf(sq / (float)D + 1e-5f);
+#pragma unroll
+                for (int ks = 0; ks < KS; ++ks) {
+                    uint4 c[2];
+#pragma unroll
+                    for (int h = 0; h < 2; ++h) {
+                        const float4 gv = *(const float4*)(c_g + 32 * ks + 16 * h + 4 * gq), bv = *(const float4*)(c_be + 32 * ks + 16 * h + 4 * gq);
+                        const f32x4 v = acc2[2 * ks + h][b];
+                        const float o[4] = {(v[0] - mean) * rstd * gv.x + bv.x, (v[1] - mean) * rstd * gv.y + bv.y, (v[2] - mean) * rstd * gv.z + bv.z,
+                                            (v[3] - mean) * rstd * gv.w + bv.w};
+                        c[h] = Chunk<T>::pack(o);
+                    }
+                    Mma<T>::regroup(c[0], c[1], xH[ks][b], xL[ks][b]);
+                }
+            }
+            wait_vm_only<0>();
+#pragma unroll
+            for (int a = 0; a < NB2; ++a)
+#pragma unroll
+                for (int b = 0; b < TB; ++b) acc2[a][b] = (f32x4){0.f, 0.f, 0.f, 0.f};
+        }
         {
             const char* const U1 = next_unit();
             g1(U1, false, bias_of(0));
@@ -250,10 +357,16 @@
             g2(second(U1));
         }
 
-        const int pn_tok = lane >> 2, pn_g = lane & 3;
-        const int pn_src = 4 * (16 * pn_g + pn_tok);
+        int le = lane;
+        int pn_tok = le >> 2, pn_g = le & 3;
+        int pn_src = 4 * (16 * pn_g + pn_tok);
 #pragma unroll
         for (int b = 0; b < TB; ++b) {
+            if constexpr (PROJ) {
+                le = lane_here();
+                pn_tok = le >> 2; pn_g = le & 3;
+                pn_src = 4 * (16 * pn_g + pn_tok);
+            }
 #pragma unroll
             for (int a = 0; a < NB2; ++a)
 #pragma unroll
@@ -261,7 +374,7 @@
                     acc2[a][b][r] = __int_as_float(__builtin_amdgcn_ds_bpermute(pn_src, __float_as_int(acc2[a][b][r])));
             const int tok = tok0 + 16 * b + pn_tok;
             const bool ok = tok < p.M;
-            float* xr = p.x + (size_t)(ok ? tok : 0) * D + 4 * pn_g;
+            float* xr = PROJ ? lane_ptr(p.x + (size_t)tile * (128 * D), ((ok ? tok - tile * 128 : 0) * D + 4 * pn_g) * 4) : p.x + (size_t)(ok ? tok : 0) * D + 4 * pn_g;
             float sum = 0.f;
             float4 rvs[NB2];
 #pragma unroll
@@ -278,20 +391,33 @@
             }
             if (p.xn) {
                 float mean = 0.f, rstd = 1.f;
-                if (next_ln) {
-                    sum += __shfl_xor(sum, 1);
-                    sum += __shfl_xor(sum, 2);
+                if (PROJ || next_ln) {
+                    if constexpr (PROJ) {
+                        sum = lane_xor_sum(sum, le, 1, 2);
+                    } else {
+                        sum += __shfl_xor(sum, 1);
+                        sum += __shfl_xor(sum, 2);
+                    }
                     mean = sum / (float)D;
                     float sq = 0.f;
 #pragma unroll
                     for (int a = 0; a < NB2; ++a)
 #pragma unroll
                         for (int r = 0; r < 4; ++r) { const float d = acc2[a][b][r] - mean; sq += d * d; }
-                    sq += __shfl_xor(sq, 1);
-                    sq += __shfl_xor(sq, 2);
+                    if constexpr (PROJ) {
+                        sq = lane_xor_sum(sq, le, 1, 2);
+                    } else {
+                        sq += __shfl_xor(sq, 1);
+                        sq += __shfl_xor(sq, 2);
+                    }
                     rstd = rsqrtf(sq / (float)D + 1e-5f);
-                }
-                T* nr = (T*)p.xn + (size_t)(ok ? tok : 0) * D + 4 * pn_g;
+                    if constexpr (PROJ) {
+                        mean = next_ln ? mean : 0.f;
+                        rstd = next_ln ? rstd : 1.f;
+                    }
+                }
+                T* nr = PROJ ? lane_ptr((T*)p.xn + (size_t)tile * (128 * D), ((ok ? tok - tile * 128 : 0) * D + 4 * pn_g) * 4)
+                             : (T*)p.xn + (size_t)(ok ? tok : 0) * D + 4 * pn_g;
 #pragma unroll
                 for (int a = 0; a < NB2; ++a) {
                     const float4 gv = *(const float4*)(c_ng + 16 * a + 4 * pn_g), bvn = *(const float4*)(c_nb + 16 * a + 4 * pn_g);
@@ -322,19 +448,27 @@
     return ldexpf(1.0f, std::min(std::max(14 - e, -100), 100));
 }
 
-void pack_mlp_x2_stream(const float* w1, const float* w2, int D, std::vector<char>& out) {
+void pack_mlp_x2_stream(const float* w1, const float* w2, int D, std::vector<char>& out, const float* wproj) {
     const int H4 = 4 * D, NCH = H4 / 32, KS = D / 32;
-    const float s1 = x2_scale(w1, (size_t)H4 * D), s2 = x2_scale(w2, (size_t)D * H4);
-    const size_t rows_per_unit = (size_t)KS * 32 + D, nrows = (size_t)(NCH + 1) * rows_per_unit;
+    const float s1 = x2_scale(w1, (size_t)H4 * D), s2 = x2_scale(w2, (size_t)D * H4), sp = wproj ? x2_scale(wproj, (size_t)D * D) : 1.f;
+    const size_t rows_per_unit = (size_t)KS * 32 + D, nrows = (size_t)(NCH + 1) * rows_per_unit + (wproj ? (size_t)KS * D : 0);
     std::vector<float> buf(nrows * 32, 0.f);
     std::vector<int> rowidx(nrows);
     size_t o = 0, ri = 0;
+    if (wproj)
+        for (int ks = 0; ks < KS; ++ks)
+            for (int n = 0; n < D; ++n) {
+                rowidx[ri++] = n;
+                for (int e = 0; e < 32; ++e, ++o) buf[o] = wproj[(size_t)n * D + 32 * ks + e] * sp;
+            }
     for (int k = 0; k <= NCH; ++k) {
         for (int ks = 0; ks < KS; ++ks)
             for (int r = 0; r < 32; ++r) {
                 rowidx[ri++] = ks * 32 + r;
-                for (int e = 0; e < 32; ++e, ++o)
-                    if (k < NCH) buf[o] = w1[(size_t)(32 * k + r) * D + 32 * ks + e] * s1;
+                for (int e = 0; e < 32; ++e, ++o) {
+                    const int ch = wproj ? 16 * ((e & 7) >> 2) + 4 * (e >> 3) + (e & 3) : e;
+                    if (k < NCH) buf[o] = w1[(size_t)(32 * k + r) * D + 32 * ks + ch] * s1;
+                }
             }
         for (int n = 0; n < D; ++n) {
             rowidx[ri++] = n;
@@ -346,7 +480,7 @@
     }
     std::vector<char> chunks(buf.size() * 4);
     convert_to_dtype(buf.data(), buf.size(), OCRVI_F16X2, chunks.data());
-    out.assign(chunks.size() + 8, 0);
+    out.assign(chunks.size() + 12, 0);
     for (size_t r = 0; r < nrows; ++r) {
         const uint64_t* src = (const uint64_t*)(chunks.data() + r * 128);
         uint64_t q[16];
@@ -360,37 +494,45 @@
             dst[2 * (ch ^ sw) + 1] = q[2 * ch + 1];
         }
     }
-    const float tail[2] = {1.0f / s1, 1.0f / s2};
-    memcpy(out.data() + chunks.size(), tail, 8);
-}
-
-template <int D, int R, int TB, bool SPLIT>
-static int launch_mlp_x2(const MlpX2Params& p, hipStream_t s) {
-    const int smem = R * (SPLIT ? 128 : 256) * D + 9 * D * 4;
-    auto kern = mlp_x2_kernel<D, R, TB, SPLIT>;
+    const float tail[3] = {1.0f / s1, 1.0f / s2, 1.0f / sp};
+    memcpy(out.data() + chunks.size(), tail, 12);
+}
+
+template <int D, int R, int TB, bool SPLIT, bool PROJ>
+static int launch_mlp_x2(const MlpX2Params& p, int grid_cap, hipStream_t s) {
+    const int smem = R * (SPLIT ? 128 : 256) * D + (PROJ ? 10 : 9) * D * 4;
+    auto kern = mlp_x2_kernel<D, R, TB, SPLIT, PROJ>;
     OCRVI_TRY(ensure_max_smem((const void*)kern, smem));
     int n_cu = 0;
     OCRVI_TRY(device_cus(&n_cu));
     const int ntiles = (p.M + 127) / 128;
     int grid = std::min(ntiles, n_cu);
     grid = cdiv(ntiles, cdiv(ntiles, grid));
+    if (grid_cap > 0) grid = std::min(grid, grid_cap);
     hipLaunchKernelGGL(kern, dim3(grid), dim3(512 / TB), smem, s, p);
     OCRVI_HIP(hipGetLastError());
     return OCRVI_OK;
 }
 
 int k_mlp_x2(float* x, void* xn, const float* ln_g, const float* ln_b, const float* next_g, const float* next_b, const void* wstream, const float* b1,
-             const float* b2, int M, int D, hipStream_t s) {
+             const float* b2, int M, int D, hipStream_t s, const MlpProj* proj, int grid_cap) {
     OCRVI_CHECK((D == 128 || D == 256 || D == 384) && x && ln_g && ln_b && wstream && b1 && b2 && M > 0 && M < (1 << 24), OCRVI_EINVAL,
                 "mlp_x2: bad argument (D %d, M %d)", D, M);
+    OCRVI_CHECK(!proj || (D != 128 && proj->a && proj->bias && proj->res), OCRVI_EINVAL, "mlp_x2: bad proj argument (D %d)", D);
     MlpX2Params p;
     p.x = x; p.xn = xn; p.ln_g = ln_g; p.ln_b = ln_b; p.next_g = next_g; p.next_b = next_b; p.wstream = (const char*)wstream; p.b1 = b1; p.b2 = b2; p.M = M;
     char tag[64];
-    snprintf(tag, sizeof(tag), "mlp_fused_d%d_f16x2", D);
+    snprintf(tag, sizeof(tag), "mlp_fused_d%d_f16x2%s", D, proj ? "_p" : "");
+    if (proj) {
+        p.a = proj->a; p.bp = proj->bias; p.xres = proj->res;
+        ProfScope ps(tag, 2.0 * M * 9.0 * D * D, (double)M * D * (20.0 + (xn ? 4.0 : 0.0)) + 9.0 * D * D * 4.0, s);
+        if (D == 256) return launch_mlp_x2<256, 2, 1, false, true>(p, grid_cap, s);
+        return launch_mlp_x2<384, 3, 2, true, true>(p, grid_cap, s);
+    }
     ProfScope ps(tag, 2.0 * M * 8.0 * D * D, (double)M * D * (8.0 + (xn ? 4.0 : 0.0)) + 8.0 * D * D * 4.0, s);
-    if (D == 128) return launch_mlp_x2<128, 4, 1, false>(p, s);
-    if (D == 256) return launch_mlp_x2<256, 2, 1, false>(p, s);
-    return launch_mlp_x2<384, 3, 2, true>(p, s);
-}
-
-}
+    if (D == 128) return launch_mlp_x2<128, 4, 1, false, false>(p, grid_cap, s);
+    if (D == 256) return launch_mlp_x2<256, 2, 1, false, false>(p, grid_cap, s);
+    return launch_mlp_x2<384, 3, 2, true, false>(p, grid_cap, s);
+}
+
+}
diff --git a/ocr_vi_invoice_amd/csrc/rec_model.hip b/ocr_vi_invoice_amd/csrc/rec_model.hip
--- a/ocr_vi_invoice_amd/csrc/rec_model.hip
+++ b/ocr_vi_invoice_amd/csrc/rec_model.hip
@@ -14,6 +14,7 @@
     ConvLayer fc1, fc2;
     void* stream = nullptr;
     float *b1 = nullptr, *b2 = nullptr;
+    float* bp = nullptr;
 };
 struct BlockW {
     bool local = false;
@@ -47,7 +48,7 @@
 static int load_lin(DeviceStore& st, const Blob& b, const std::string& name, int cout, int cin, int dt, ConvLayer* L, const float* extra = nullptr) {
     return load_conv(st, b, name, cout, cin, 0, 1, AM_CONV1, dt, true, L, extra);
 }
-static int load_mlp(DeviceStore& st, const Blob& b, const std::string& name, int d, int dt, MlpW* m) {
+static int load_mlp(DeviceStore& st, const Blob& b, const std::string& name, int d, int dt, MlpW* m, const std::string& proj = "") {
     OCRVI_TRY(load_lin(st, b, name + ".fc1", 4 * d, d, dt, &m->fc1));
     OCRVI_TRY(load_lin(st, b, name + ".fc2", d, 4 * d, dt, &m->fc2));
     static const bool fuse = !(getenv("OCRVI_MLP_FUSED") && atoi(getenv("OCRVI_MLP_FUSED")) == 0);
@@ -58,7 +59,15 @@
         OCRVI_TRY(b.get(name + ".fc2.w", d, 4 * d, 0, 0, &w2));
         OCRVI_TRY(b.get(name + ".fc2.b", d, 0, 0, 0, &b2));
         std::vector<char> packed;
-        pack_mlp_stream(w1->data, w2->data, d, dt, packed);
+        if (!proj.empty() && dt == OCRVI_F16X2 && d == 384) {
+            const BlobTensor *wp = nullptr, *bp = nullptr;
+            OCRVI_TRY(b.get(proj + ".w", d, d, 0, 0, &wp));
+            OCRVI_TRY(b.get(proj + ".b", d, 0, 0, 0, &bp));
+            pack_mlp_x2_stream(w1->data, w2->data, d, packed, wp->data);
+            OCRVI_TRY(st.upload(bp->data, (size_t)d * 4, (void**)&m->bp));
+        } else {
+            pack_mlp_stream(w1->data, w2->data, d, dt, packed);
+        }
         OCRVI_TRY(st.upload(packed.data(), packed.size(), &m->stream));
         OCRVI_TRY(st.upload(b1->data, (size_t)4 * d * 4, (void**)&m->b1));
         OCRVI_TRY(st.upload(b2->data, (size_t)d * 4, (void**)&m->b2));
@@ -104,7 +113,7 @@
                 OCRVI_TRY(load_lin(st, blob, p + ".mixer.qkv", 3 * d, d, dt, &bw.qkv));
                 OCRVI_TRY(load_lin(st, blob, p + ".mixer.proj", d, d, dt, &bw.proj));
             }
-            OCRVI_TRY(load_mlp(st, blob, p + ".mlp", d, dt, &bw.mlp));
+            OCRVI_TRY(load_mlp(st, blob, p + ".mlp", d, dt, &bw.mlp, bw.local ? "" : p + ".mixer.proj"));
         }
         if (s < 2) OCRVI_TRY(load_conv(st, blob, "merges." + std::to_string(s), cfg->dims[s + 1], d, 3, 1, AM_CONV3, dt, true, &h->merge[s]));
     }
@@ -120,7 +129,7 @@
     const BlobTensor* tok = nullptr;
     OCRVI_TRY(blob.get("frm.select_token", d, 0, 0, 0, &tok));
     OCRVI_TRY(load_lin(st, blob, "frm.v_proj", d, d, dt, &h->v_proj, tok->data));
-    OCRVI_TRY(load_mlp(st, blob, "frm.h_mlp", d, dt, &h->h_mlp));
+    OCRVI_TRY(load_mlp(st, blob, "frm.h_mlp", d, dt, &h->h_mlp, "frm.h_proj"));
     OCRVI_TRY(load_mlp(st, blob, "frm.v_mlp", d, dt, &h->v_mlp));
     OCRVI_TRY(load_vec(st, blob, "frm.vq", d, &h->vq));
     OCRVI_TRY(load_lin(st, blob, "head", cfg->num_classes, d, dt, &h->head));
@@ -161,12 +170,19 @@
 
 static const LNw kCast{};
 static int mlp_block(Runner& r, const Tensor& x, const Tensor& xn, const Tensor& hb, const LNw& n, const MlpW& m, int d, const LNw* next = nullptr,
-                     bool* xn_done = nullptr) {
+                     bool* xn_done = nullptr, const Tensor* pa = nullptr, const Tensor* pres = nullptr) {
     const int rows = (int)x.pixels();
     if (xn_done) *xn_done = false;
+    OCRVI_CHECK((m.bp != nullptr) == (pa != nullptr && pres != nullptr), OCRVI_EINVAL, "mlp_block: the projection's operands do not match the packed stream");
     if (m.stream) {
         if (xn_done) *xn_done = next != nullptr;
         if (r.dry()) return OCRVI_OK;
+        if (m.bp) {
+            MlpProj pj;
+            pj.a = pa->p; pj.bias = m.bp; pj.res = (const float*)pres->p;
+            return k_mlp_x2((float*)x.p, next ? xn.p : nullptr, n.g, n.b, next ? next->g : nullptr, next ? next->b : nullptr, m.stream, m.b1, m.b2, rows, d,
+                            r.stream, &pj);
+        }
         return k_mlp_fused(r.dtype, (float*)x.p, next ? xn.p : nullptr, n.g, n.b, next ? next->g : nullptr, next ? next->b : nullptr, m.stream, m.b1, m.b2,
                            rows, d, r.stream);
     }
@@ -241,10 +257,12 @@
                 OCRVI_TRY(conv(r, bw.qkv, view(xn, rows, 1, 1, d), view(big, rows, 1, 1, 3 * d), o));
                 OCRVI_TRY(attention(r, big, t1, B, Hs * Ws, d / 32));
                 o.res = &xs; o.res_mode = RES_SAME;
-                OCRVI_TRY(conv(r, bw.proj, view(t1, rows, 1, 1, d), view(xs, rows, 1, 1, d), o));
+                if (!bw.mlp.bp) OCRVI_TRY(conv(r, bw.proj, view(t1, rows, 1, 1, d), view(xs, rows, 1, 1, d), o));
             }
             const LNw* next = bi + 1 < nblk ? &h->blocks[s][bi + 1].n1 : ((s < 2 && lowp) ? &kCast : nullptr);
-            OCRVI_TRY(mlp_block(r, view(xs, rows, 1, 1, d), xn, big, bw.n2, bw.mlp, d, next, &xn_ready));
+            const Tensor xrows = view(xs, rows, 1, 1, d), arows = view(t1, rows, 1, 1, d);
+            const bool pj = bw.mlp.bp != nullptr;
+            OCRVI_TRY(mlp_block(r, xrows, xn, big, bw.n2, bw.mlp, d, next, &xn_ready, pj ? &arows : nullptr, pj ? &xrows : nullptr));
         }
         if (s < 2) {
             Tensor src = xn;
@@ -274,10 +292,13 @@
         OCRVI_TRY(conv(r, h->h_qkv, xn, view(big, rows, 1, 1, 3 * d2), o));
         OCRVI_TRY(attention(r, big, t1, B * Hs, Ws, d2 / 32));
         o.res = &bn; o.res_mode = RES_SAME;
-        OCRVI_TRY(conv(r, h->h_proj, t1, xr, o));
+        if (!h->h_mlp.bp) OCRVI_TRY(conv(r, h->h_proj, t1, xr, o));
     }
     bool xn_ready = false;
-    OCRVI_TRY(mlp_block(r, xr, xn, big, h->h_norm2, h->h_mlp, d2, &h->v_norm_kv, &xn_ready));
+    {
+        const bool pj = h->h_mlp.bp != nullptr;
+        OCRVI_TRY(mlp_block(r, xr, xn, big, h->h_norm2, h->h_mlp, d2, &h->v_norm_kv, &xn_ready, pj ? &t1 : nullptr, pj ? &bn : nullptr));
+    }
     if (!xn_ready) OCRVI_TRY(ln(r, xr, xn, h->v_norm_kv));
     const int cols = B * Ws;
     const Tensor tq = wrap(r.arena.alloc((size_t)cols * d2 * 4), cols, 1, 1, d2, true);
```

Result: no change. 326.6 (-0.3%).
